# koide3/hdl_graph_slam

Hardware: AMD Instinct MI355X
Metric: registrations/sec (64-beam ~120k-pt pair), loop-closure batch (higher is better)
Workload: dtype f64; 1 GPU; loop-closure batch: 64 candidate keyframes/GPU x HDL-64E (~118848 pts) vs 1 query keyframe, FAST_GICP + getFitnessScore, cold (index + covariances rebuilt every step); candidate set: SURVEY 8d (distinct ray-casts at poses within 20 m of the query, guess = ground truth + 0.5 m / 2 deg noise, z forced to 0); candidates_per_gpu=64, points_per_cloud=118848, method=FAST_GICP, distinct_scans=16, parallelism=single GPU

## Files before the change

### hdl_graph_slam_amd/_lib.py

```python
from __future__ import annotations

import ctypes as C
import os

import numpy as np

_HERE = os.path.dirname(os.path.abspath(__file__))
LIB_PATH = os.path.join(_HERE, "lib", "libhgs_hip.so")

HGS_OK = 0
HGS_ERR_INVALID_ARGUMENT, HGS_ERR_NO_TARGET, HGS_ERR_NO_SOURCE, HGS_ERR_HIP, HGS_ERR_NO_DEVICE, HGS_ERR_UNSUPPORTED, HGS_ERR_OUT_OF_MEMORY, HGS_ERR_INTERNAL, HGS_ERR_COMM = range(1, 10)
HGS_FAST_GICP, HGS_FAST_VGICP, HGS_NDT_OMP, HGS_ICP = 0, 1, 2, 3
HGS_KDTREE, HGS_DIRECT1, HGS_DIRECT7, HGS_DIRECT27 = 0, 1, 2, 3
HGS_REG_FROBENIUS, HGS_REG_PLANE, HGS_REG_MIN_EIG, HGS_REG_NORMALIZED_MIN_EIG, HGS_REG_NONE = 0, 1, 2, 3, 4
STAGES = ["upload", "index", "covariance", "voxelize", "linearize", "error", "solve", "fitness", "prefilter"]
DBL_MAX = float(np.finfo(np.float64).max)

STATUS = {1: "invalid argument", 2: "no target set", 3: "no source set", 4: "HIP runtime error", 5: "no usable HIP device", 6: "unsupported",
          7: "out of host memory inside the backend", 8: "internal error (C++ exception caught at the C boundary)", 9: "communicator error (RCCL)"}


class HgsParams(C.Structure):
    _fields_ = [
        ("method", C.c_int32), ("max_iterations", C.c_int32),
        ("transformation_epsilon", C.c_double), ("rotation_epsilon", C.c_double),
        ("max_correspondence_distance", C.c_double),
        ("correspondence_randomness", C.c_int32), ("neighbor_search", C.c_int32),
        ("resolution", C.c_double), ("ndt_step_size", C.c_double), ("ndt_outlier_ratio", C.c_double),
        ("ndt_min_points_per_voxel", C.c_int32), ("ndt_upstream_hd1_sign", C.c_int32),
        ("lm_max_iterations", C.c_int32), ("lm_init_lambda_factor", C.c_double),
        ("device_id", C.c_int32), ("regularization_method", C.c_int32),
        ("ndt_line_search", C.c_int32), ("reserved", C.c_int32),
    ]

    @property
    def use_reciprocal_correspondences(self) -> bool:
        return bool(self.reserved)

    @use_reciprocal_correspondences.setter
    def use_reciprocal_correspondences(self, on: bool) -> None:
        self.reserved = 1 if on else 0


class HgsPrefilterParams(C.Structure):
    _fields_ = [
        ("use_distance_filter", C.c_int32), ("downsample_method", C.c_int32),
        ("distance_near_thresh", C.c_double), ("distance_far_thresh", C.c_double), ("downsample_resolution", C.c_double),
        ("outlier_removal_method", C.c_int32), ("statistical_mean_k", C.c_int32),
        ("statistical_stddev", C.c_double), ("radius_radius", C.c_double),
        ("radius_min_neighbors", C.c_int32), ("reserved", C.c_int32),
    ]


class HgsPrefilterSweep(C.Structure):
    _fields_ = [
        ("pts", C.c_void_p), ("n", C.c_size_t), ("stride_bytes", C.c_size_t),
        ("imu_angular_velocity", C.c_void_p), ("scan_period", C.c_double), ("sensor_to_base", C.c_void_p),
    ]


class HgsFloorParams(C.Structure):
    _fields_ = [
        ("tilt_deg", C.c_double), ("sensor_height", C.c_double), ("height_clip_range", C.c_double),
        ("floor_pts_thresh", C.c_int32), ("use_normal_filtering", C.c_int32),
        ("floor_normal_thresh", C.c_double), ("normal_filter_thresh", C.c_double),
        ("normal_k", C.c_int32), ("ransac_max_iterations", C.c_int32),
        ("ransac_distance_threshold", C.c_double), ("ransac_probability", C.c_double),
        ("seed", C.c_uint32), ("reserved", C.c_int32),
    ]


class HgsFloorResult(C.Structure):
    _fields_ = [
        ("coeffs", C.c_float * 4), ("detected", C.c_int32), ("reason", C.c_int32),
        ("n_clipped", C.c_uint32), ("n_filtered", C.c_uint32), ("n_inliers", C.c_uint32), ("ransac_iterations", C.c_int32),
    ]


HGS_FLOOR_DETECTED, HGS_FLOOR_TOO_FEW_POINTS, HGS_FLOOR_TOO_FEW_INLIERS, HGS_FLOOR_NOT_VERTICAL = 0, 1, 2, 3
HGS_DOWNSAMPLE_NONE, HGS_DOWNSAMPLE_VOXELGRID, HGS_DOWNSAMPLE_APPROX_VOXELGRID = 0, 1, 2
HGS_OUTLIER_NONE, HGS_OUTLIER_STATISTICAL, HGS_OUTLIER_RADIUS = 0, 1, 2


class HgsResult(C.Structure):
    _fields_ = [
        ("final_transformation", C.c_float * 16), ("converged", C.c_int32), ("iterations", C.c_int32),
        ("error", C.c_double), ("fitness_score", C.c_double), ("num_inliers", C.c_uint32),
        ("candidate_id", C.c_int32), ("lm_tries", C.c_int32), ("reserved", C.c_int32),
    ]

    def matrix(self) -> np.ndarray:
        return np.array(self.final_transformation, dtype=np.float32).reshape(4, 4).T.copy()


RESULT_DTYPE = np.dtype([("final_transformation", "<f4", (16,)), ("converged", "<i4"), ("iterations", "<i4"), ("error", "<f8"),
                         ("fitness_score", "<f8"), ("num_inliers", "<u4"), ("candidate_id", "<i4"), ("lm_tries", "<i4"), ("reserved", "<i4")])
assert RESULT_DTYPE.itemsize == C.sizeof(HgsResult)

EXPORTS = [
    "hgs_params_default", "hgs_create", "hgs_destroy", "hgs_last_error", "hgs_abi_version",
    "hgs_cloud_create", "hgs_cloud_destroy", "hgs_cloud_size", "hgs_cloud_device_bytes", "hgs_cloud_invalidate",
    "hgs_set_target", "hgs_set_target_cloud", "hgs_set_source", "hgs_set_source_cloud",
    "hgs_align", "hgs_transform_source", "hgs_fitness", "hgs_nn_target",
    "hgs_loop_match_batch", "hgs_loop_match_groups", "hgs_align_pairs", "hgs_select_best", "hgs_calc_fitness_score", "hgs_calc_fitness_score_batch",
    "hgs_comm_get_unique_id", "hgs_comm_init", "hgs_comm_finalize", "hgs_loop_match_batch_sharded",
    "hgs_prefilter_params_default", "hgs_prefilter", "hgs_prefilter_deskewed", "hgs_prefilter_framed", "hgs_prefilter_batch", "hgs_cloud_download", "hgs_map_cloud_generate",
    "hgs_floor_params_default", "hgs_detect_floor", "hgs_debug_floor_filter", "hgs_debug_floor_ransac_counts",
    "hgs_profile_enable", "hgs_profile_read", "hgs_synchronize",
    "hgs_debug_target_covariances", "hgs_debug_gicp_linearize", "hgs_debug_icp_correspond", "hgs_debug_icp_step", "hgs_debug_ndt_cells", "hgs_debug_vgicp_voxels", "hgs_debug_cloud_seed_grid", "hgs_debug_ndt_derivatives", "hgs_debug_merge_shard_records", "hgs_debug_set_option",
]

_lib = None


def lib():
    global _lib
    if _lib is not None:
        return _lib
    if not os.path.exists(LIB_PATH):
        raise RuntimeError(f"{LIB_PATH} is missing: build the MI355X backend first (python -c 'import __graft_entry__ as g; g.build()'). "
                           "hdl_graph_slam_amd has no CPU fallback.")
    L = C.CDLL(LIB_PATH)
    vp, sz, fp = C.c_void_p, C.c_size_t, C.POINTER(C.c_float)
    L.hgs_params_default.argtypes = [C.c_int32, C.POINTER(HgsParams)]
    L.hgs_create.argtypes = [C.POINTER(HgsParams), C.POINTER(vp)]
    L.hgs_destroy.argtypes = [vp]
    L.hgs_last_error.argtypes = [vp]
    L.hgs_last_error.restype = C.c_char_p
    L.hgs_cloud_create.argtypes = [vp, vp, sz, sz, C.POINTER(vp)]
    L.hgs_cloud_destroy.argtypes = [vp]
    L.hgs_cloud_size.argtypes = [vp]
    L.hgs_cloud_size.restype = sz
    L.hgs_cloud_device_bytes.argtypes = [vp]
    L.hgs_cloud_device_bytes.restype = sz
    L.hgs_cloud_invalidate.argtypes = [vp]
    L.hgs_set_target.argtypes = [vp, vp, sz, sz]
    L.hgs_set_source.argtypes = [vp, vp, sz, sz]
    L.hgs_set_target_cloud.argtypes = [vp, vp]
    L.hgs_set_source_cloud.argtypes = [vp, vp]
    L.hgs_align.argtypes = [vp, fp, C.POINTER(HgsResult)]
    L.hgs_transform_source.argtypes = [vp, fp, vp, sz]
    L.hgs_fitness.argtypes = [vp, fp, C.c_double, C.POINTER(C.c_double), C.POINTER(C.c_uint32)]
    L.hgs_nn_target.argtypes = [vp, vp, sz, sz, vp, vp]
    L.hgs_loop_match_batch.argtypes = [vp, C.POINTER(vp), sz, vp, C.c_double, vp, C.POINTER(C.c_int32)]
    L.hgs_loop_match_groups.argtypes = [vp, C.POINTER(vp), sz, vp, C.POINTER(vp), vp, C.c_double, vp, vp]
    L.hgs_align_pairs.argtypes = [vp, C.POINTER(vp), C.POINTER(vp), vp, C.POINTER(C.c_double), sz, vp]
    L.hgs_select_best.argtypes = [vp, sz, C.POINTER(C.c_int32)]
    L.hgs_comm_get_unique_id.argtypes = [vp]
    L.hgs_comm_init.argtypes = [vp, C.c_int32, C.c_int32, vp]
    L.hgs_comm_finalize.argtypes = [vp]
    L.hgs_loop_match_batch_sharded.argtypes = [vp, C.POINTER(vp), sz, vp, vp, sz, C.c_double, vp, C.POINTER(C.c_int32)]
    L.hgs_calc_fitness_score.argtypes = [vp, vp, vp, fp, C.c_double, C.POINTER(C.c_double)]
    L.hgs_calc_fitness_score_batch.argtypes = [vp, C.POINTER(vp), C.POINTER(vp), vp, sz, C.c_double, vp, vp]
    L.hgs_prefilter_params_default.argtypes = [C.POINTER(HgsPrefilterParams)]
    L.hgs_prefilter.argtypes = [vp, vp, sz, sz, C.POINTER(HgsPrefilterParams), C.POINTER(vp)]
    L.hgs_prefilter_deskewed.argtypes = [vp, vp, sz, sz, C.POINTER(HgsPrefilterParams), vp, C.c_double, C.POINTER(vp)]
    L.hgs_prefilter_framed.argtypes = [vp, vp, sz, sz, C.POINTER(HgsPrefilterParams), vp, C.c_double, fp, C.POINTER(vp)]
    L.hgs_prefilter_batch.argtypes = [vp, C.POINTER(HgsPrefilterSweep), sz, C.POINTER(HgsPrefilterParams), C.POINTER(vp)]
    L.hgs_cloud_download.argtypes = [vp, vp, sz]
    L.hgs_map_cloud_generate.argtypes = [vp, C.POINTER(vp), vp, sz, C.c_double, C.POINTER(vp)]
    L.hgs_floor_params_default.argtypes = [C.POINTER(HgsFloorParams)]
    L.hgs_detect_floor.argtypes = [vp, vp, C.POINTER(HgsFloorParams), C.POINTER(HgsFloorResult), C.POINTER(vp), C.POINTER(vp)]
    L.hgs_debug_floor_filter.argtypes = [vp, vp, C.POINTER(HgsFloorParams), vp, vp, vp]
    L.hgs_debug_floor_ransac_counts.argtypes = [vp, vp, C.POINTER(HgsFloorParams), C.c_uint32, C.c_uint32, vp, vp]
    L.hgs_profile_enable.argtypes = [vp, C.c_int]
    L.hgs_profile_read.argtypes = [vp, vp, vp, C.c_int]
    L.hgs_synchronize.argtypes = [vp]
    L.hgs_debug_target_covariances.argtypes = [vp, vp]
    L.hgs_debug_set_option.argtypes = [vp, C.c_char_p, C.c_int32]
    L.hgs_debug_gicp_linearize.argtypes = [vp, vp, vp, vp, vp, vp]
    L.hgs_debug_icp_correspond.argtypes = [vp, vp, vp, vp]
    L.hgs_debug_icp_step.argtypes = [vp, vp, vp, C.c_double, C.c_int32, vp, vp, vp]
    L.hgs_debug_ndt_cells.argtypes = [vp, C.c_int32, vp, vp, vp, vp, C.POINTER(C.c_int32)]
    L.hgs_debug_vgicp_voxels.argtypes = [vp, C.c_int32, vp, vp, vp, vp, C.POINTER(C.c_int32)]
    L.hgs_debug_cloud_seed_grid.argtypes = [vp, vp, vp, sz, C.POINTER(C.c_int32), C.POINTER(sz)]
    L.hgs_debug_ndt_derivatives.argtypes = [vp, vp, vp, vp, vp]
    L.hgs_debug_merge_shard_records.argtypes = [vp, vp, C.c_int32, C.c_size_t, C.c_size_t, vp, vp]
    _lib = L
    return L


def default_params(method: int) -> HgsParams:
    p = HgsParams()
    rc = lib().hgs_params_default(method, C.byref(p))
    if rc != HGS_OK:
        raise ValueError(f"hgs_params_default({method}) -> {STATUS.get(rc, rc)}")
    return p


def cloud_args(cloud: np.ndarray):
    cloud = np.ascontiguousarray(cloud)
    if cloud.dtype.fields is not None:
        return cloud, len(cloud), cloud.dtype.itemsize
    cloud = np.ascontiguousarray(cloud, dtype=np.float32)
    if cloud.ndim != 2 or cloud.shape[1] < 3:
        raise ValueError("expected [n, >=3] float32 or PointXYZI records")
    return cloud, cloud.shape[0], cloud.shape[1] * 4


def colmajor16(T) -> np.ndarray:
    return np.ascontiguousarray(np.asarray(T, dtype=np.float32).reshape(4, 4).T.reshape(16))


def fptr(a: np.ndarray):
    return a.ctypes.data_as(C.POINTER(C.c_float))
```

### hdl_graph_slam_amd/csrc/hgs_device.h

```cpp
#pragma once
#include <hip/hip_runtime.h>
#include "hgs_gicp.h"
#include "hgs_floor.h"
#include "hgs_icp.h"
#include "hgs_ndt.h"
#include "hgs_vgicp.h"

namespace hgs {

struct CloudMeta {
  int nvalid;
  int ndt_ncells;
  unsigned bbmin[3];
  unsigned bbmax[3];
  int ndt_min_b[3], ndt_max_b[3], ndt_div_mul[3];
  int ndt_error;
  int vg_ncells;
  int vg_min_b[3], vg_max_b[3], vg_div_mul[3];
  int vg_error;
  int pad[1];
};

struct CloudDesc {
  const float4* raw;
  float4* pts;
  float4* lpts;
  float4* nodes;
  float4* cov;
  int* corr;
  CloudMeta* meta;
  int n_input;
  int P;
  int sort_off;
  int pad;
};

struct TargetView {
  const float4* nodes;
  const float4* pts;
  const float4* lpts;
  const float4* cov;
  const CloudMeta* meta;
  int P;
  int seed_bits;
  const unsigned* seed_tab;
};

struct NdtTargetView {
  const int* hash_keys;
  const int* hash_vals;
  const NdtCellRec* cells;
  const CloudMeta* meta;
  const int2* hash_kv;
  int hash_mask;
  float inv_leaf;
};

struct NdtAccum {
  unsigned long long w[kAccNdt * 4];
  unsigned tiles_done;
  unsigned overflow;
  double out[kAccNdt];
};

struct DevResult {
  float T[16];
  int converged, iterations, lm_tries, pad;
  double error;
  double fit_sum;
  unsigned fit_count;
  unsigned pad2;
};

struct Progress {
  int* dev;
  volatile int* host_done;
  volatile int* host_rounds;
  int B;
  int pad;
};

constexpr int kFusedRoundMaxProblems = 4;
constexpr int kBlock = 256;
constexpr int kKnnLaneList = 16;
constexpr int kKnnLeafLog = 128;
constexpr int kNW = 1;
constexpr int kTileNN = kBlock * kNW;

void launch_pack_aos(hipStream_t s, const float4* staged , int n, float4* raw, float* intensity , CloudMeta* meta_to_reset ,
                     const CloudDesc* desc = nullptr , CloudDesc* desc_out = nullptr);
void launch_meta_init(hipStream_t s, const CloudDesc* descs, int ncloud);
void launch_bbox_count(hipStream_t s, const CloudDesc* descs, int ncloud, int max_n);
void launch_hilbert_keys(hipStream_t s, const CloudDesc* descs, int ncloud, int max_n, unsigned long long* keys, unsigned* vals, int drop_bits);
void launch_gather_sorted(hipStream_t s, const CloudDesc* descs, int ncloud, int max_slots, const unsigned* sorted_vals);
void launch_build_tree(hipStream_t s, const CloudDesc* descs, int ncloud, int max_P);
void launch_knn_cov(hipStream_t s, const CloudDesc* descs, int ncloud, int max_n, int k, int qpw, int reg_method, int gather ,
                    double* raw_stage = nullptr );

void launch_gicp_init(hipStream_t s, GicpState* states, const float* guesses, int B, Progress prog);
struct Guess16 {
  float m[16];
};
void launch_gicp_init1(hipStream_t s, GicpState* states, const float* guess_host , Progress prog);
void launch_gicp_linearize(hipStream_t s, const CloudDesc* descs, TargetView tgt, const GicpState* states, GicpConsts c, double* partials, int max_blocks, int B,
                           int qpw);
void launch_gicp_solve(hipStream_t s, const CloudDesc* descs, GicpState* states, GicpConsts c, const double* partials, int max_blocks, int B,
                       int tile_points );
void launch_gicp_error(hipStream_t s, const CloudDesc* descs, TargetView tgt, const GicpState* states, double* partials_err, int max_blocks, int B);
void launch_gicp_linearize_round2(hipStream_t s, const CloudDesc* descs, TargetView tgt, const GicpState* states_in, GicpState* states_out, GicpConsts c, double* partials,
                                  const double* partials_err, int max_blocks , int lin_blocks , int B, int qpw, Progress prog,
                                  DevResult* results, DevResult* early_out );
void launch_gicp_error_round2(hipStream_t s, const CloudDesc* descs, TargetView tgt, const GicpState* states_in, GicpState* states_out, GicpConsts c, const double* partials,
                              double* partials_err, int max_blocks, int err_blocks , int B, int lin_tile_points);
void launch_gicp_decide(hipStream_t s, const CloudDesc* descs, GicpState* states, GicpConsts c, const double* partials_err, int max_blocks, int B, Progress prog);
void launch_gicp_results(hipStream_t s, const GicpState* states, DevResult* out, int B);

void launch_icp_init(hipStream_t s, IcpState* states, const float* guesses, int B, Progress prog);
void launch_icp_correspond(hipStream_t s, const CloudDesc* descs, TargetView tgt, const IcpState* states, IcpConsts c, double* partials, int max_blocks, int B);
void launch_icp_solve(hipStream_t s, const CloudDesc* descs, IcpState* states, IcpConsts c, const double* partials, int max_blocks, int B, Progress prog);
void launch_icp_results(hipStream_t s, const IcpState* states, DevResult* out, int B);

void launch_fitness(hipStream_t s, const CloudDesc* descs, TargetView tgt, const DevResult* poses, double max_range, double* partials, int max_blocks, int B,
                    int use_seed, int qpw);
void launch_fitness_final(hipStream_t s, const CloudDesc* descs, const double* partials, int max_blocks, DevResult* out, int B, int tile_pts);
void launch_gicp_linearize(hipStream_t s, const CloudDesc* descs, const TargetView* tviews, const GicpState* states, GicpConsts c, double* partials, int max_blocks, int B,
                           int qpw);
void launch_gicp_error(hipStream_t s, const CloudDesc* descs, const TargetView* tviews, const GicpState* states, double* partials_err, int max_blocks, int B);
void launch_gicp_linearize_round2(hipStream_t s, const CloudDesc* descs, const TargetView* tviews, const GicpState* states_in, GicpState* states_out, GicpConsts c, double* partials,
                                  const double* partials_err, int max_blocks, int lin_blocks, int B, int qpw, Progress prog, DevResult* results, DevResult* early_out);
void launch_gicp_error_round2(hipStream_t s, const CloudDesc* descs, const TargetView* tviews, const GicpState* states_in, GicpState* states_out, GicpConsts c, const double* partials,
                              double* partials_err, int max_blocks, int err_blocks, int B, int lin_tile_points);
void launch_icp_correspond(hipStream_t s, const CloudDesc* descs, const TargetView* tviews, const IcpState* states, IcpConsts c, double* partials, int max_blocks, int B);
void launch_fitness(hipStream_t s, const CloudDesc* descs, const TargetView* tviews, const DevResult* poses, double max_range, double* partials, int max_blocks, int B,
                    int use_seed, int qpw);
}
struct hgs_result;
namespace hgs {
void launch_results_to_records(hipStream_t s, const DevResult* res, const int* candidate_ids, int n, int n_slots, ::hgs_result* out);
void launch_nn_query(hipStream_t s, TargetView tgt, const float4* q, int nq, int* idx, float* d2);
void launch_seed_grid_build(hipStream_t s, const float4* pts, const CloudMeta* meta, int n_max, unsigned* tab, int bits);
inline size_t seed_grid_entries(int bits) { return ((size_t)1 << bits) + ((size_t)1 << (bits - 2)) + ((size_t)1 << (bits - 4)); }
struct SeedGridJob {
  const float4* pts;
  const CloudMeta* meta;
  unsigned* tab;
  int bits;
  int pad;
};
void launch_seed_grid_build_batch(hipStream_t s, const SeedGridJob* jobs, int njobs, size_t max_entries, int max_n);
void launch_transform(hipStream_t s, const float4* raw, int n, const float* T16_colmajor_dev, float4* out);

void launch_ndt_grid_params(hipStream_t s, CloudDesc desc, float inv_leaf);
void launch_ndt_cell_keys(hipStream_t s, CloudDesc desc, float inv_leaf, unsigned long long* keys, unsigned* vals);
void launch_ndt_build_cells(hipStream_t s, CloudDesc desc, const unsigned long long* sorted_keys, const unsigned* sorted_vals, int min_points,
                            int* hash_keys, int* hash_vals, int hash_mask, NdtCellRec* cells);
void launch_ndt_init(hipStream_t s, NdtState* states, NdtAngles* angles, const float* guesses, NdtConsts c, int B, Progress prog, NdtAccum* accum_to_zero );
void launch_ndt_pack_hash(hipStream_t s, const int* keys, const int* vals, int2* kv, int cap);
void launch_ndt_pass(hipStream_t s, const CloudDesc* descs, NdtTargetView tgt, NdtState* states, NdtAngles* angles, NdtConsts c, NdtAccum* accum, const int* tile_base,
                     unsigned long long* queues, int B, int parity, int blocks, int chunk, int sorted, int debug, Progress prog);
void launch_ndt_pass(hipStream_t s, const CloudDesc* descs, const NdtTargetView* tviews, NdtState* states, NdtAngles* angles, NdtConsts c, NdtAccum* accum, const int* tile_base,
                     unsigned long long* queues, int B, int parity, int blocks, int chunk, int sorted, int debug, Progress prog);
void launch_ndt_results(hipStream_t s, const CloudDesc* descs, const NdtState* states, DevResult* out, int B);

void launch_vgicp_grid_params(hipStream_t s, CloudDesc desc, double resolution);
void launch_vgicp_cell_keys(hipStream_t s, CloudDesc desc, double resolution, unsigned long long* keys, unsigned* vals);
void launch_vgicp_build_cells(hipStream_t s, CloudDesc desc, const unsigned long long* sorted_keys, const unsigned* sorted_vals, int* hash_keys,
                              int* hash_vals, int hash_mask, NdtCellRec* cells);
void launch_vgicp_linearize(hipStream_t s, const CloudDesc* descs, NdtTargetView tgt, const GicpState* states, VgicpConsts c, double* partials,
                            int max_blocks, int B);
void launch_vgicp_error(hipStream_t s, const CloudDesc* descs, NdtTargetView tgt, const GicpState* states, VgicpConsts c, double* partials_err,
                        int max_blocks, int B);
void launch_vgicp_linearize(hipStream_t s, const CloudDesc* descs, const NdtTargetView* tviews, const GicpState* states, VgicpConsts c, double* partials,
                            int max_blocks, int B);
void launch_vgicp_error(hipStream_t s, const CloudDesc* descs, const NdtTargetView* tviews, const GicpState* states, VgicpConsts c, double* partials_err,
                        int max_blocks, int B);

struct MapSource {
  const float4* raw;
  const float* intensity;
  int n, offset;
  float T[16];
};
void launch_map_transform(hipStream_t s, const MapSource* srcs, int nsrc, int max_n, float4* out);
constexpr int kMapMaxDepth = 21;
constexpr int kMapMaxEvents = kMapMaxDepth + 3;
struct MapOctreeEvent {
  int index, depth;
  double mn[3];
  unsigned long long gained[3];
};
struct MapOctree {
  int first;
  int next_viol;
  int n_events, overflow, done, pad;
  double mx[3];
  MapOctreeEvent events[kMapMaxEvents];
};
void launch_map_first_finite(hipStream_t s, const float4* pts, int n, MapOctree* oct);
void launch_map_octree_init(hipStream_t s, const float4* pts, int n, double res, MapOctree* oct);
void launch_map_octree_step(hipStream_t s, const float4* pts, int n, double res, MapOctree* oct);
void launch_map_keys(hipStream_t s, const float4* pts, int n, double res, const MapOctree* oct, unsigned long long* keys, unsigned* vals);
void launch_map_centers(hipStream_t s, const unsigned long long* keys, const unsigned* head, const unsigned* slot, int n, double res, const MapOctree* oct, float4* out,
                        int* count_out);

struct PfFrame {
  float rows[12];
};
void launch_pf_load(hipStream_t s, const float4* staged, int n, float4* out, const float* deskew_w , double scan_period,
                    const PfFrame* frame , int* count_out, unsigned* meta_out );
void launch_pf_distance_flags(hipStream_t s, const float4* pts, int n, int use_filter, double near_thresh, double far_thresh, unsigned* keep);
void launch_pf_compact(hipStream_t s, const float4* in, int n, const unsigned* keep, const unsigned* slot, float4* out, int* count);
void launch_pf_bbox(hipStream_t s, const float4* pts, const int* count, int cap, unsigned* meta, int dist_filter = 0, double near_thresh = 0, double far_thresh = 0);
void launch_pf_grid(hipStream_t s, unsigned* meta, float inv_leaf);
void launch_pf_voxel_keys(hipStream_t s, const float4* pts, const int* count, const unsigned* meta, float inv_leaf, int cap, unsigned long long* keys, unsigned* vals,
                          int dist_filter = 0, double near_thresh = 0, double far_thresh = 0);
void launch_pf_voxel_heads(hipStream_t s, const unsigned long long* keys, int cap, unsigned* head, unsigned long long invalid_key);
constexpr unsigned long long kVoxelInvalidKey = 0xffffffffull;
constexpr unsigned long long kMapInvalidKey = ~0ull;
void launch_pf_voxel_centroids(hipStream_t s, const float4* pts, const unsigned long long* keys, const unsigned* vals, const unsigned* head, const unsigned* slot, int cap,
                               float4* out, int* count_out, unsigned* ukeys = nullptr );
void launch_pf_grid_radius_flags(hipStream_t s, const float4* cen, const int* count, const unsigned* ukeys, const unsigned* meta, float inv_leaf, float radius, float r2,
                                 int min_neighbors, int cap, unsigned* keep);
void launch_pf_approx_keys(hipStream_t s, const float4* pts, const int* count, float inv_leaf, int cap, unsigned long long* keys, unsigned* vals);
void launch_pf_approx_heads(hipStream_t s, const float4* pts, const unsigned long long* keys, const unsigned* vals, float inv_leaf, int cap, unsigned* head, unsigned* evict,
                            unsigned* bucket_used , unsigned* bucket_rank );
void launch_pf_approx_centroids(hipStream_t s, const float4* pts, const unsigned long long* keys, const unsigned* vals, const unsigned* head, const unsigned* evict,
                                const unsigned* evict_rank, const unsigned* bucket_rank, int cap, float4* out, int* count_out);
void launch_pf_radius_flags(hipStream_t s, CloudDesc d, float r2, int min_neighbors, unsigned* keep);
void launch_pf_mean_knn_dist(hipStream_t s, CloudDesc d, int mean_k, double* dist);
void launch_pf_statistical(hipStream_t s, CloudDesc d, const double* dist, double* stats, double stddev_mul, unsigned* keep);
void launch_pf_to_cloud(hipStream_t s, const float4* in, int n, float4* raw, float* intensity, CloudMeta* meta_to_reset, const CloudDesc* desc = nullptr, CloudDesc* desc_out = nullptr);

struct PfSweep {
  int off, n;
  int count;
  int deskew, frame;
  float w[3];
  double scan_period;
  float rows[12];
  unsigned meta[16];
};
constexpr int kPfBatchOrdinalBits = 12;
void launch_pfb_load(hipStream_t s, const float4* staged, PfSweep* sweeps, int nsweeps, int max_n, float4* out);
void launch_pfb_distance_flags(hipStream_t s, const float4* pts, const PfSweep* sweeps, int nsweeps, int max_n, double near_thresh, double far_thresh, unsigned* keep);
void launch_pfb_compact(hipStream_t s, const float4* in, PfSweep* sweeps, int nsweeps, int max_n, const unsigned* keep, const unsigned* slot, float4* out);
void launch_pfb_bbox(hipStream_t s, const float4* pts, PfSweep* sweeps, int nsweeps, int max_n, int dist_filter, double near_thresh, double far_thresh);
void launch_pfb_grid(hipStream_t s, PfSweep* sweeps, int nsweeps, float inv_leaf);
void launch_pfb_voxel_keys(hipStream_t s, const float4* pts, const PfSweep* sweeps, int nsweeps, int max_n, float inv_leaf, unsigned long long* keys, unsigned* vals,
                           int dist_filter, double near_thresh, double far_thresh);
void launch_pfb_voxel_heads(hipStream_t s, const unsigned long long* keys, const PfSweep* sweeps, int nsweeps, int max_n, unsigned* head);
void launch_pfb_voxel_centroids(hipStream_t s, const float4* pts, const unsigned long long* keys, const unsigned* vals, const unsigned* head, const unsigned* slot,
                                PfSweep* sweeps, int nsweeps, int max_n, float4* out, unsigned* ukeys );
void launch_pfb_grid_radius_flags(hipStream_t s, const float4* cen, const unsigned* ukeys, const PfSweep* sweeps, int nsweeps, int max_n, float inv_leaf, float radius,
                                  float r2, int min_neighbors, unsigned* keep);
void launch_pfb_to_cloud(hipStream_t s, const float4* in, const PfSweep* sweeps, const CloudDesc* descs, CloudDesc* const* desc_outs, float* const* intensities, int nsweeps,
                         int max_m);

void launch_floor_clip_flags(hipStream_t s, const float4* raw, const float* intensity, int n, FloorConsts c, float4* out , unsigned* keep);
void launch_knn_cov_raw(hipStream_t s, const CloudDesc* descs , int max_n, int k, int qpw, int gather, double* raw_stage );
void launch_floor_normal_flags(hipStream_t s, CloudDesc d, const double* raw_cov, FloorConsts c, unsigned* keep , double* normals );
void launch_floor_ransac_init(hipStream_t s, FloorRansacState* st, int max_iterations, Progress prog);
void launch_floor_ransac_planes(hipStream_t s, const float4* pts, int n, unsigned seed, int i0, int nh, const FloorRansacState* st , double* planes ,
                                int* counts );
void launch_floor_ransac_count(hipStream_t s, const float4* pts, int n, double thresh, const double* planes, int nh, const FloorRansacState* st , int* counts);
void launch_floor_ransac_decide(hipStream_t s, const int* counts, const double* planes, int i0, int nh, int n, int max_iterations, double log_prob, FloorRansacState* st,
                                Progress prog);
void launch_floor_inlier_flags(hipStream_t s, const float4* pts, int n, const FloorRansacState* st, double thresh, unsigned* keep);

void launch_gicp_debug_state(hipStream_t s, GicpState* st, const double* T12_dev);
void launch_ndt_debug_state(hipStream_t s, NdtState* st, NdtAngles* ang, const double* p6_dev, NdtConsts c);
void launch_reduce_partials(hipStream_t s, const double* partials, int ntiles, int width , double* out);

}
```

### hdl_graph_slam_amd/csrc/hgs_engine.hip

```cpp
#include <hip/hip_runtime.h>
#include <algorithm>
#include <atomic>
#include <chrono>
#include <climits>
#include <condition_variable>
#include <cmath>
#include <cstdio>
#include <cstdlib>
#include <cstring>
#include <exception>
#include <limits>
#include <mutex>
#include <new>
#include <stdexcept>
#include <string>
#include <thread>
#include <vector>

#include "../../include/hgs_registration.h"
#include "hgs_comm.h"
#include "hgs_consts.h"
#include "hgs_device.h"
#include "hgs_resources.h"
#include "hgs_sort.h"

using namespace hgs;

namespace {

thread_local std::string g_create_error;


int next_pow2(int v) {
  int p = 1;
  while (p < v) p <<= 1;
  return p;
}
size_t align_up(size_t v, size_t a) { return (v + a - 1) / a * a; }

}

struct VoxelTable {
  DeviceBuffer block;
  int* hash_keys = nullptr;
  int* hash_vals = nullptr;
  int2* hash_kv = nullptr;
  NdtCellRec* cells = nullptr;
  int hash_cap = 0;
};

struct hgs_cloud {
  hgs_handle* owner = nullptr;
  size_t n_input = 0;
  int P = 1;
  DeviceBuffer block;
  CloudDesc desc{};
  CloudDesc* dev_desc = nullptr;
  float* intensity = nullptr;
  bool has_index = false;
  bool corr_stale = false;
  bool has_cov = false;
  int cov_k = 0;
  bool has_ndt = false;
  double ndt_resolution = 0;
  int ndt_min_points = 0;
  VoxelTable ndt;
  bool has_vg = false;
  double vg_resolution = 0;
  int vg_cov_k = 0;
  long long vg_span[3] = {0, 0, 0};
  bool vg_too_large = false;
  VoxelTable vg;
  bool has_seed = false;
  DeviceBuffer seed_block;
  int seed_bits = 0;
};

struct ProfEvent {
  int stage;
  hipEvent_t a, b;
};

struct hgs_handle {
  hgs_params prm{};
  int device = 0;
  hipStream_t stream = nullptr;
  hipStream_t lane_stream[7] = {};
  hipEvent_t lane_event[8] = {};
  int lane_start = 1;
  int nn_qpw = 0;
  int nn_qpw16_below = 96, nn_qpw32_below = 0;
  int hilbert_levels = 13;
  hipEvent_t comm_event = nullptr;
  int prefilter_fast = 1;
  int upload_trace = 0;
  int floor_chunk = 64;
  int early_run_ahead = 2;
  int early_result = 1;
  PinnedBuffer h_early;
  hipEvent_t early_event = nullptr;
  bool early_pending = false, early_valid = false;
  int fused_rounds = 1;
  int fused_rounds_below = 262144;
  int fused_rounds_max_problems = kFusedRoundMaxProblems, fused_rounds_max_blocks = 640;
  int cov_split = 1;
  int resident_descs = 1;
  int knn_qpw_tiny = -1;
  int knn_tiny_below = 32768;
  int seed_grid = 1;
  int knn_replay = -1;
  int batch_lanes = 0;
  std::string err;
  hgs_cloud* target = nullptr;
  hgs_cloud* source = nullptr;
  bool own_target = false, own_source = false;
  float final_T[16];

  DeviceBuffer staging, sort_keys[2], sort_vals[2], sort_tmp, descs, states, angles, partials, partials_err, results, guesses, done, misc;
  DeviceBuffer lane_partials[7], lane_partials_err[7];
  DeviceBuffer ndt_accum;
  DeviceBuffer group_tviews, group_corr;
  DeviceBuffer group_vviews;
  DeviceBuffer seed_jobs;
  int pair_chunk = 0;
  hgs::Comm* comm = nullptr;
  DeviceBuffer comm_send, comm_recv, comm_ids;
  DeviceBuffer pf_ukeys;
  DeviceBuffer cov_raw;
  DeviceBuffer ndt_plan;
  int ndt_resident_blocks = 0;
  int ndt_chunk = 0;
  int ndt_sort = -1;
  DeviceBuffer pf_a, pf_b, pf_keep, pf_slot, pf_small, pf_dist;
  DeviceBuffer pf_table;
  PinnedBuffer h_pf_table;
  PinnedBuffer h_results, h_small, h_flags, h_comm;
  PinnedRing up;
  PinnedRing up_points;
  PinnedBuffer up_big;
  hipEvent_t up_big_event = nullptr;
  bool up_big_pending = false;
  PackPool pack_pool;
  PinnedBuffer h_xform;

  std::vector<DeviceBuffer> block_pool;
  std::vector<hgs_cloud*> live_clouds;
  std::recursive_mutex api_mutex;

  bool profiling = false;
  std::vector<ProfEvent> prof_events;
  std::vector<ProfEvent> prof_free;
  double prof_ms[HGS_STAGE_COUNT];
  uint64_t prof_launches[HGS_STAGE_COUNT];

  hgs_handle() = default;
  hgs_handle(const hgs_handle&) = delete;
  hgs_handle& operator=(const hgs_handle&) = delete;
  void synchronize_streams() {
    if (stream) (void)hipStreamSynchronize(stream);
    for (hipStream_t ls : lane_stream)
      if (ls) (void)hipStreamSynchronize(ls);
  }
  ~hgs_handle();
};

namespace {

#define HGS_HIP(h, call)                                                                                           \
  do {                                                                                                             \
    hipError_t e__ = (call);                                                                                       \
    if (e__ != hipSuccess) {                                                                                       \
      char buf__[512];                                                                                             \
      snprintf(buf__, sizeof(buf__), "%s failed: %s (%s:%d)", #call, hipGetErrorString(e__), __FILE__, __LINE__);  \
      (h)->err = buf__;                                                                                            \
      return HGS_ERR_HIP;                                                                                          \
    }                                                                                                              \
  } while (0)

#define HGS_TRY(expr)             \
  do {                            \
    int rc__ = (expr);            \
    if (rc__ != HGS_OK) return rc__; \
  } while (0)

struct StageTimer {
  hgs_handle* h;
  ProfEvent ev{};
  bool active = false;
  StageTimer(hgs_handle* h_, int stage) : h(h_) {
    if (!h->profiling) return;
    if (!h->prof_free.empty()) {
      ev = h->prof_free.back();
      h->prof_free.pop_back();
    } else {
      if (hipEventCreate(&ev.a) != hipSuccess || hipEventCreate(&ev.b) != hipSuccess) return;
    }
    ev.stage = stage;
    active = hipEventRecord(ev.a, h->stream) == hipSuccess;
  }
  ~StageTimer() {
    if (!active) return;
    (void)hipEventRecord(ev.b, h->stream);
    h->prof_events.push_back(ev);
  }
};

struct ApiLock {
  std::unique_lock<std::recursive_mutex> lk;
  explicit ApiLock(hgs_handle* h) {
    if (h) lk = std::unique_lock<std::recursive_mutex>(h->api_mutex);
  }
  explicit ApiLock(hgs_cloud* c) : ApiLock(c ? c->owner : nullptr) {}
};

int set_device(hgs_handle* h) {
  HGS_HIP(h, hipSetDevice(h->device));
  return HGS_OK;
}

constexpr size_t kUploadChunkPoints = 16384;
#ifndef HGS_UPLOAD_PARALLEL_POINTS
#define HGS_UPLOAD_PARALLEL_POINTS 49152
#endif
constexpr size_t kUploadParallelPoints = HGS_UPLOAD_PARALLEL_POINTS;
int upload_image_open(hgs_handle* h, size_t records) {
  if (h->up_big_pending) {
    HGS_HIP(h, hipEventSynchronize(h->up_big_event));
    h->up_big_pending = false;
  }
  HGS_HIP(h, h->up_big.reserve(records * sizeof(float4)));
  return HGS_OK;
}
int upload_image_close(hgs_handle* h) {
  if (!h->up_big_event) HGS_HIP(h, hipEventCreateWithFlags(&h->up_big_event, hipEventDisableTiming));
  HGS_HIP(h, hipEventRecord(h->up_big_event, h->stream));
  h->up_big_pending = true;
  return HGS_OK;
}
int upload_points_at(hgs_handle* h, const void* pts, size_t n, size_t stride_bytes, size_t off, bool in_image) {
  const bool has_intensity = stride_bytes >= 20;
  const char* src = static_cast<const char*>(pts);
  float4* const dev = h->staging.as<float4>() + off;
  if (n >= kUploadParallelPoints) {
    if (!in_image) HGS_TRY(upload_image_open(h, n));
    float4* const image = h->up_big.as<float4>() + (in_image ? off : 0);
    const size_t nchunks = (n + kUploadChunkPoints - 1) / kUploadChunkPoints;
    std::vector<std::atomic<unsigned char>> ready(nchunks);
    for (auto& r : ready) r.store(0, std::memory_order_relaxed);
    PackPool::Job job;
    job.src = src, job.dst = reinterpret_cast<float*>(image), job.n = n, job.stride = stride_bytes, job.chunk = kUploadChunkPoints, job.nchunks = nchunks;
    job.has_intensity = has_intensity, job.ready = ready.data();
    h->pack_pool.post(&job);
    hipError_t err = hipSuccess;
    for (size_t c = 0; c < nchunks; c++) {
      while (!ready[c].load(std::memory_order_acquire))
        if (!PackPool::help(job)) std::this_thread::yield();
      const size_t i0 = c * kUploadChunkPoints, m = std::min(kUploadChunkPoints, n - i0);
      if (err == hipSuccess) err = hipMemcpyAsync(dev + i0, image + i0, m * sizeof(float4), hipMemcpyHostToDevice, h->stream);
    }
    h->pack_pool.retire();
    HGS_HIP(h, err);
    if (!in_image) HGS_TRY(upload_image_close(h));
    return HGS_OK;
  }
  for (size_t i0 = 0; i0 < n; i0 += kUploadChunkPoints) {
    const size_t m = std::min(kUploadChunkPoints, n - i0);
    void* staged = nullptr;
    int slot = 0;
    HGS_HIP(h, h->up_points.stage(kUploadChunkPoints * sizeof(float4), &staged, &slot));
    float* dst = static_cast<float*>(staged);
    const char* s0 = src + i0 * stride_bytes;
    if (has_intensity) {
      for (size_t i = 0; i < m; i++) {
        const float* f = reinterpret_cast<const float*>(s0 + i * stride_bytes);
        dst[4 * i] = f[0], dst[4 * i + 1] = f[1], dst[4 * i + 2] = f[2], dst[4 * i + 3] = f[4];
      }
    } else {
      for (size_t i = 0; i < m; i++) {
        const float* f = reinterpret_cast<const float*>(s0 + i * stride_bytes);
        dst[4 * i] = f[0], dst[4 * i + 1] = f[1], dst[4 * i + 2] = f[2], dst[4 * i + 3] = 0.f;
      }
    }
    HGS_HIP(h, hipMemcpyAsync(dev + i0, staged, m * sizeof(float4), hipMemcpyHostToDevice, h->stream));
    HGS_HIP(h, h->up_points.commit(slot, h->stream));
  }
  return HGS_OK;
}
int upload_points_packed(hgs_handle* h, const void* pts, size_t n, size_t stride_bytes, const float4** dev) {
  HGS_HIP(h, h->staging.reserve(std::max<size_t>(n, 1) * sizeof(float4)));
  *dev = h->staging.as<float4>();
  return upload_points_at(h, pts, n, stride_bytes, 0, false);
}

int cloud_alloc(hgs_handle* h, size_t n, hgs_cloud** out) {
  hgs_cloud* c = new hgs_cloud();
  c->owner = h;
  c->n_input = n;
  c->P = next_pow2((int)((n + kLeaf - 1) / kLeaf));
  if (c->P < 1) c->P = 1;
  const size_t slots = (size_t)c->P * kLeaf;
  const size_t n_cap = align_up(std::max<size_t>(n, 1), 8192);
  size_t off = 0;
  const size_t o_meta = off;
  off = align_up(off + sizeof(CloudMeta), 256);
  const size_t o_desc = off;
  off = align_up(off + sizeof(CloudDesc), 256);
  const size_t o_raw = off;
  off = align_up(off + n_cap * sizeof(float4), 256);
  const size_t o_pts = off;
  off = align_up(off + slots * sizeof(float4), 256);
  const size_t o_lpts = off;
  off = align_up(off + slots * sizeof(float4), 256);
  const size_t o_nodes = off;
// ... 239 lines not shown
      [&](unsigned long long* keys, unsigned* vals) { launch_ndt_build_cells(h->stream, c->desc, keys, vals, min_pts, t.hash_keys, t.hash_vals, cap - 1, t.cells); }));
  launch_ndt_pack_hash(h->stream, t.hash_keys, t.hash_vals, t.hash_kv, cap);
  HGS_HIP(h, hipGetLastError());
  c->has_ndt = true;
  c->ndt_resolution = res;
  c->ndt_min_points = min_pts;
  return HGS_OK;
}

int vgicp_grid_too_large(hgs_handle* h, const hgs_cloud* c) {
  char msg[256];
  snprintf(msg, sizeof(msg),
           "FAST_VGICP: the target's voxel grid spans %lld x %lld x %lld cells at resolution %g, more than the 2147483647 a linear voxel key addresses "
           "(a far stray point in the target?)",
           c->vg_span[0], c->vg_span[1], c->vg_span[2], c->vg_resolution);
  h->err = msg;
  return HGS_ERR_UNSUPPORTED;
}

int ensure_vgicp_target(hgs_handle* h, hgs_cloud* c) {
  const double res = h->prm.resolution;
  const int k = h->prm.correspondence_randomness;
  if (c->has_vg && c->vg_resolution == res && c->vg_cov_k == cov_cache_key(h, k)) return c->vg_too_large ? vgicp_grid_too_large(h, c) : HGS_OK;
  StageTimer tm(h, HGS_STAGE_VOXELIZE);
  const int max_cells = (int)c->n_input + 1;
  const int cap = next_pow2(std::max<int>(64, 2 * max_cells));
  VoxelTable& t = c->vg;
  HGS_TRY(build_voxel_table(
      h, c, t, cap, max_cells, false, [&] { launch_vgicp_grid_params(h->stream, c->desc, res); },
      [&](unsigned long long* keys, unsigned* vals) { launch_vgicp_cell_keys(h->stream, c->desc, res, keys, vals); },
      [&](unsigned long long* keys, unsigned* vals) { launch_vgicp_build_cells(h->stream, c->desc, keys, vals, t.hash_keys, t.hash_vals, cap - 1, t.cells); }));
  HGS_HIP(h, hipGetLastError());
  HGS_HIP(h, h->h_small.reserve(sizeof(CloudMeta)));
  const CloudMeta* hm = h->h_small.as<CloudMeta>();
  HGS_HIP(h, hipMemcpyAsync(h->h_small.p, c->desc.meta, sizeof(CloudMeta), hipMemcpyDeviceToHost, h->stream));
  HGS_HIP(h, hipStreamSynchronize(h->stream));
  for (int d = 0; d < 3; d++) c->vg_span[d] = (long long)hm->vg_max_b[d] - hm->vg_min_b[d] + 1;
  c->vg_too_large = hm->vg_error != 0;
  c->has_vg = true;
  c->vg_resolution = res;
  c->vg_cov_k = cov_cache_key(h, k);
  return c->vg_too_large ? vgicp_grid_too_large(h, c) : HGS_OK;
}

NdtTargetView voxel_target_view(const hgs_cloud* c, const VoxelTable& t, float inv_leaf) {
  NdtTargetView tv;
  tv.hash_keys = t.hash_keys, tv.hash_vals = t.hash_vals, tv.cells = t.cells, tv.meta = c->desc.meta, tv.hash_kv = t.hash_kv;
  tv.hash_mask = t.hash_cap - 1, tv.inv_leaf = inv_leaf;
  return tv;
}
NdtTargetView ndt_target_view(const hgs_handle* h, const hgs_cloud* t) { return voxel_target_view(t, t->ndt, 1.0f / (float)h->prm.resolution); }
NdtTargetView vgicp_target_view(const hgs_cloud* t) { return voxel_target_view(t, t->vg, 0.f); }

TargetView target_view(const hgs_cloud* c) {
  TargetView t;
  t.nodes = c->desc.nodes, t.pts = c->desc.pts, t.lpts = c->desc.lpts, t.cov = c->desc.cov, t.meta = c->desc.meta, t.P = c->P;
  t.seed_bits = c->has_seed ? c->seed_bits : 0, t.seed_tab = c->has_seed ? c->seed_block.as<const unsigned>() : nullptr;
  return t;
}

int ensure_seed_grid(hgs_handle* h, hgs_cloud* c) {
  if (!h->seed_grid || c->has_seed || !c->has_index || c->n_input == 0) return HGS_OK;
  int bits = 12;
  while (bits < 24 && ((size_t)1 << bits) < 4 * c->n_input) bits++;
  const size_t bytes = seed_grid_entries(bits) * sizeof(unsigned);
  if (!c->seed_block.p || c->seed_bits != bits) {
    HGS_HIP(h, c->seed_block.alloc(bytes));
    c->seed_bits = bits;
  }
  HGS_HIP(h, hipMemsetAsync(c->seed_block.p, 0xff, bytes, h->stream));
  launch_seed_grid_build(h->stream, c->desc.pts, c->desc.meta, (int)c->n_input, c->seed_block.as<unsigned>(), bits);
  HGS_HIP(h, hipGetLastError());
  c->has_seed = true;
  return HGS_OK;
}

int ensure_seed_grids(hgs_handle* h, const std::vector<hgs_cloud*>& all) {
  if (!h->seed_grid) return HGS_OK;
  std::vector<hgs_cloud*> todo;
  for (hgs_cloud* c : all)
    if (!c->has_seed && c->has_index && c->n_input > 0 && std::find(todo.begin(), todo.end(), c) == todo.end()) todo.push_back(c);
  constexpr size_t kMaxJobs = 65535;
  for (size_t start = 0; start < todo.size(); start += kMaxJobs) {
    const size_t nj = std::min(kMaxJobs, todo.size() - start);
    std::vector<SeedGridJob> jobs(nj);
    size_t max_entries = 0;
    int max_n = 0;
    for (size_t j = 0; j < nj; j++) {
      hgs_cloud* c = todo[start + j];
      int bits = 12;
      while (bits < 24 && ((size_t)1 << bits) < 4 * c->n_input) bits++;
      const size_t entries = seed_grid_entries(bits);
      if (!c->seed_block.p || c->seed_bits != bits) {
        HGS_HIP(h, c->seed_block.alloc(entries * sizeof(unsigned)));
        c->seed_bits = bits;
      }
      jobs[j] = SeedGridJob{c->desc.pts, c->desc.meta, c->seed_block.as<unsigned>(), bits, 0};
      max_entries = std::max(max_entries, entries), max_n = std::max(max_n, (int)c->n_input);
    }
    HGS_HIP(h, h->seed_jobs.reserve(nj * sizeof(SeedGridJob)));
    HGS_HIP(h, h->up.upload(h->seed_jobs.p, jobs.data(), nj * sizeof(SeedGridJob), h->stream));
    launch_seed_grid_build_batch(h->stream, h->seed_jobs.as<SeedGridJob>(), (int)nj, max_entries, max_n);
    HGS_HIP(h, hipGetLastError());
    for (size_t j = 0; j < nj; j++) todo[start + j]->has_seed = true;
  }
  return HGS_OK;
}

NdtConsts engine_ndt_consts(const hgs_params& p) {
  NdtConsts c = ndt_consts(p);
  c.pad = std::getenv("HGS_TRACE") ? 1 : 0;
  return c;
}

constexpr int kMaxCountedDevices = 64;
std::atomic<int> g_streams_in_use[kMaxCountedDevices] = {};
std::atomic<int>& streams_in_use(int device) { return g_streams_in_use[(unsigned)device % kMaxCountedDevices]; }
int hw_queue_budget() {
  static const int budget = [] {
    const char* e = std::getenv("GPU_MAX_HW_QUEUES");
    const int v = e ? std::atoi(e) : 0;
    return v > 0 ? v : 4;
  }();
  return budget;
}
constexpr int kFloorMaxChunk = 4096;
constexpr int kMaxLanes = 8;

int make_progress(hgs_handle* h, int lane, int B, Progress* out) {
  if (h->early_pending) {
    HGS_HIP(h, hipEventSynchronize(h->early_event));
    h->early_pending = false;
  }
  HGS_HIP(h, h->done.reserve(64));
  HGS_HIP(h, h->h_flags.reserve(64));
  volatile int* hf = h->h_flags.as<volatile int>() + 2 * lane;
  hf[0] = 0, hf[1] = 0;
  out->dev = h->done.as<int>() + 2 * lane;
  out->host_done = hf, out->host_rounds = hf + 1;
  out->B = B, out->pad = 0;
  return HGS_OK;
}

struct BatchLane {
  hipStream_t stream = nullptr;
  int b0 = 0, B = 0;
  Progress prog{};
  double* partials = nullptr;
  double* partials_err = nullptr;
  long round = 0;
  bool finished = false;
};

int open_lanes(hgs_handle* h, int B, size_t partial_bytes_per_problem, size_t partial_err_bytes_per_problem, std::vector<BatchLane>& lanes, int tiles_per_problem) {
  const bool small_problems = tiles_per_problem > 0 && tiles_per_problem <= 96;
  const int by_size = h->prm.method == HGS_NDT_OMP ? (B > 32 && !small_problems ? 3 : 4) : (small_problems && (long)B * tiles_per_problem <= 3072 ? 1 : 4);
  const int wanted = h->batch_lanes > 0 ? h->batch_lanes : by_size;
  int n = h->profiling ? 1 : std::max(1, std::min(std::min(wanted, kMaxLanes), B));
  if (h->batch_lanes <= 0) {
    int owned = 0;
    while (owned < kMaxLanes - 1 && h->lane_stream[owned]) owned++;
    const int room = std::max(0, hw_queue_budget() - streams_in_use(h->device).load(std::memory_order_relaxed));
    n = std::min(n, 1 + owned + room);
  }
  lanes.assign(n, BatchLane{});
  for (int i = 0, b0 = 0; i < n; i++) {
    BatchLane& L = lanes[i];
    L.b0 = b0, L.B = (B - b0) / (n - i);
    b0 += L.B;
    HGS_TRY(make_progress(h, i, L.B, &L.prog));
    if (i == 0) {
      L.stream = h->stream;
      L.partials = h->partials.as<double>(), L.partials_err = h->partials_err.as<double>();
      continue;
    }
    if (!h->lane_stream[i - 1]) {
      HGS_HIP(h, hipStreamCreateWithFlags(&h->lane_stream[i - 1], hipStreamNonBlocking));
      streams_in_use(h->device).fetch_add(1, std::memory_order_relaxed);
    }
    L.stream = h->lane_stream[i - 1];
    HGS_HIP(h, h->lane_partials[i - 1].reserve((size_t)L.B * partial_bytes_per_problem));
    HGS_HIP(h, h->lane_partials_err[i - 1].reserve((size_t)L.B * partial_err_bytes_per_problem));
    L.partials = h->lane_partials[i - 1].as<double>(), L.partials_err = h->lane_partials_err[i - 1].as<double>();
  }
  if (n > 1) {
    if (h->lane_start != 0) HGS_HIP(h, hipStreamSynchronize(h->stream));
    if (!h->lane_event[0]) HGS_HIP(h, hipEventCreateWithFlags(&h->lane_event[0], hipEventDisableTiming));
    HGS_HIP(h, hipEventRecord(h->lane_event[0], h->stream));
    for (int i = 1; i < n; i++) HGS_HIP(h, hipStreamWaitEvent(lanes[i].stream, h->lane_event[0], 0));
  }
  return HGS_OK;
}

int close_lanes(hgs_handle* h, std::vector<BatchLane>& lanes) {
  for (size_t i = 1; i < lanes.size(); i++) {
    if (!h->lane_event[i]) HGS_HIP(h, hipEventCreateWithFlags(&h->lane_event[i], hipEventDisableTiming));
    HGS_HIP(h, hipEventRecord(h->lane_event[i], lanes[i].stream));
    HGS_HIP(h, hipStreamWaitEvent(h->stream, h->lane_event[i], 0));
  }
  return HGS_OK;
}

constexpr long kRunAhead = 2;
template <typename F, typename G>
void drive_lanes(std::vector<BatchLane>& lanes, long max_rounds, F&& enqueue_round, G&& on_finished, long run_ahead = kRunAhead) {
  long spins = 0;
  for (;;) {
    bool all_finished = true, enqueued = false;
    for (BatchLane& L : lanes) {
      if (L.finished) continue;
      if (*L.prog.host_done || L.round >= max_rounds) {
        L.finished = true;
        on_finished(L);
        continue;
      }
      all_finished = false;
      if (L.round - (long)*L.prog.host_rounds < run_ahead) {
        enqueue_round(L);
        L.round++;
        enqueued = true;
      }
    }
    if (all_finished) return;
    if (enqueued) {
      spins = 0;
      continue;
    }
    if ((++spins & 0x3ff) == 0) {
      for (BatchLane& L : lanes)
        if (!L.finished && !*L.prog.host_done && hipStreamQuery(L.stream) == hipSuccess && !*L.prog.host_done &&
            L.round - (long)*L.prog.host_rounds >= run_ahead) {
          enqueue_round(L);
          L.round++;
        }
    }
#if defined(__x86_64__)
    __builtin_ia32_pause();
#endif
  }
}

struct BatchShape {
  int B, max_n;
  int qpw, nn_tile;
  bool gicp_round2;
  int lin_qpw, lin_tile, lin_blocks;
  int max_blocks, err_blocks;
  const CloudDesc* d_descs;
  const TargetView* d_tviews;
  const NdtTargetView* d_vviews;
};

template <typename F>
void with_lane_target(const BatchShape& s, const BatchLane& L, const TargetView& tv, F&& launch) {
  if (s.d_tviews) launch(s.d_tviews + L.b0);
  else launch(tv);
}

int batch_shape(hgs_handle* h, const std::vector<hgs_cloud*>& sources, bool lm_rounds, BatchShape* out, int* const* corr_of = nullptr) {
  BatchShape& s = *out;
  s.d_tviews = nullptr, s.d_vviews = nullptr;
  s.B = (int)sources.size();
  s.max_n = 0;
  for (hgs_cloud* c : sources) s.max_n = std::max(s.max_n, (int)c->n_input);
  const int B = s.B, max_n = s.max_n;
  s.qpw = 64;
  s.nn_tile = (kBlock / 64) * s.qpw * kNW;
  s.gicp_round2 = lm_rounds && h->prm.method == HGS_FAST_GICP && h->fused_rounds && max_n <= h->fused_rounds_below &&
                  (B <= h->fused_rounds_max_problems || (long)B * ((max_n + kBlock - 1) / kBlock) <= (long)h->fused_rounds_max_blocks);
  const long tiles64 = (long)B * ((max_n + s.nn_tile - 1) / s.nn_tile);
  s.lin_qpw = !s.gicp_round2 ? 64 : h->nn_qpw > 0 ? h->nn_qpw : tiles64 <= (long)h->nn_qpw16_below ? 16 : tiles64 <= (long)h->nn_qpw32_below ? 32 : 64;
  s.lin_tile = (kBlock / 64) * s.lin_qpw * kNW;
  s.lin_blocks = std::max(1, (max_n + s.lin_tile - 1) / s.lin_tile);
  s.max_blocks = std::max(1, s.lin_qpw < 64 ? (max_n + 63) / 64 : (max_n + s.nn_tile - 1) / s.nn_tile);
  s.err_blocks = std::max(1, (max_n + kBlock - 1) / kBlock);
  return upload_descs(h, sources, false, &s.d_descs, nullptr, corr_of);
}

bool corr_seeds_fitness(int method) { return method == HGS_FAST_GICP || method == HGS_ICP; }
void lane_fitness(hgs_handle* h, BatchLane& L, const BatchShape& s, double max_range, bool corr_seeds) {
  StageTimer tm(h, HGS_STAGE_FITNESS);
  DevResult* res = h->results.as<DevResult>() + L.b0;
  with_lane_target(s, L, s.d_tviews ? TargetView{} : target_view(h->target),
                   [&](auto tgt) { launch_fitness(L.stream, s.d_descs + L.b0, tgt, res, max_range, L.partials_err, s.max_blocks, L.B, corr_seeds ? 1 : 0, s.qpw); });
  launch_fitness_final(L.stream, s.d_descs + L.b0, L.partials_err, s.max_blocks, res, L.B, s.nn_tile);
}
void lane_fitness_tail(hgs_handle* h, BatchLane& L, const BatchShape& s, const double* fit_max_range) {
  if (fit_max_range) lane_fitness(h, L, s, *fit_max_range, corr_seeds_fitness(h->prm.method));
}

int run_gicp_rounds(hgs_handle* h, const BatchShape& s, const float* guesses_host, bool guess_in_args, const double* fit_max_range) {
  const int B = s.B, max_blocks = s.max_blocks;
  hgs_cloud* tgt = h->target;
  const bool voxel = h->prm.method == HGS_FAST_VGICP;
  const GicpConsts c = gicp_consts(h->prm);
  const VgicpConsts vc = vgicp_consts(h->prm);
  const bool round2 = s.gicp_round2;
  const bool early = round2 && B == 1 && !fit_max_range && h->early_result && !h->profiling;
  DevResult* early_out = nullptr;
  if (early) {
    HGS_HIP(h, h->h_early.reserve(sizeof(DevResult)));
    early_out = h->h_early.as<DevResult>();
  }
  HGS_HIP(h, h->states.reserve((size_t)B * sizeof(GicpState) * (round2 ? 2 : 1)));
  GicpState* st = h->states.as<GicpState>();
  GicpState* st_other = st + B;
  const TargetView tv = s.d_tviews || s.d_vviews ? TargetView{} : target_view(tgt);
  const NdtTargetView vtv = voxel && !s.d_vviews ? vgicp_target_view(tgt) : NdtTargetView{};
  const long max_rounds = (long)std::max(1, c.max_iterations) * std::max(1, c.lm_max_iterations) + 2 + (round2 ? 1 : 0);
  std::vector<BatchLane> lanes;
  HGS_TRY(open_lanes(h, B, (size_t)max_blocks * kAccNdt * sizeof(double), (size_t)max_blocks * 2 * sizeof(double), lanes, s.err_blocks));
  auto finish_lane = [&](BatchLane& L) {
    if (early && *L.prog.host_done) {
      h->early_valid = true;
      return;
    }
    launch_gicp_results(L.stream, st + L.b0, h->results.as<DevResult>() + L.b0, L.B);
    lane_fitness_tail(h, L, s, fit_max_range);
  };
  if (guess_in_args) launch_gicp_init1(lanes[0].stream, st, guesses_host, lanes[0].prog);
  else
    for (BatchLane& L : lanes) launch_gicp_init(L.stream, st + L.b0, h->guesses.as<float>() + (size_t)L.b0 * 16, L.B, L.prog);
  drive_lanes(lanes, max_rounds, [&](BatchLane& L) {
    const CloudDesc* dd = s.d_descs + L.b0;
    GicpState* ls = st + L.b0;
    if (round2) {
      {
        StageTimer tm(h, HGS_STAGE_LINEARIZE);
        with_lane_target(s, L, tv, [&](auto t) {
          launch_gicp_linearize_round2(L.stream, dd, t, ls, st_other + L.b0, c, L.partials, L.partials_err, max_blocks, s.lin_blocks, L.B, s.lin_qpw, L.prog,
                                       h->results.as<DevResult>() + L.b0, early_out);
        });
      }
      StageTimer tm(h, HGS_STAGE_ERROR);
      with_lane_target(s, L, tv, [&](auto t) {
        launch_gicp_error_round2(L.stream, dd, t, st_other + L.b0, ls, c, L.partials, L.partials_err, max_blocks, s.err_blocks, L.B, s.lin_tile);
      });
      return;
    }
    {
      StageTimer tm(h, HGS_STAGE_LINEARIZE);
      if (voxel && s.d_vviews) launch_vgicp_linearize(L.stream, dd, s.d_vviews + L.b0, ls, vc, L.partials, max_blocks, L.B);
      else if (voxel) launch_vgicp_linearize(L.stream, dd, vtv, ls, vc, L.partials, max_blocks, L.B);
      else with_lane_target(s, L, tv, [&](auto t) { launch_gicp_linearize(L.stream, dd, t, ls, c, L.partials, max_blocks, L.B, s.qpw); });
    }
    {
      StageTimer tm(h, HGS_STAGE_SOLVE);
      launch_gicp_solve(L.stream, dd, ls, c, L.partials, max_blocks, L.B, voxel ? kBlock : s.nn_tile);
    }
    {
      StageTimer tm(h, HGS_STAGE_ERROR);
      if (voxel && s.d_vviews) launch_vgicp_error(L.stream, dd, s.d_vviews + L.b0, ls, vc, L.partials_err, max_blocks, L.B);
      else if (voxel) launch_vgicp_error(L.stream, dd, vtv, ls, vc, L.partials_err, max_blocks, L.B);
      else with_lane_target(s, L, tv, [&](auto t) { launch_gicp_error(L.stream, dd, t, ls, L.partials_err, max_blocks, L.B); });
    }
    {
      StageTimer tm(h, HGS_STAGE_SOLVE);
      launch_gicp_decide(L.stream, dd, ls, c, L.partials_err, max_blocks, L.B, L.prog);
    }
  }, finish_lane, early ? (long)h->early_run_ahead : kRunAhead);
  HGS_TRY(close_lanes(h, lanes));
  if (h->early_valid) {
    if (!h->early_event) HGS_HIP(h, hipEventCreateWithFlags(&h->early_event, hipEventDisableTiming));
    HGS_HIP(h, hipEventRecord(h->early_event, h->stream));
    h->early_pending = true;
  }
  return HGS_OK;
}

int run_icp_rounds(hgs_handle* h, const BatchShape& s, const double* fit_max_range) {
  const int B = s.B, max_blocks = s.max_blocks;
  const IcpConsts c = icp_consts(h->prm);
  HGS_HIP(h, h->states.reserve((size_t)B * sizeof(IcpState)));
  IcpState* st = h->states.as<IcpState>();
  const TargetView tv = s.d_tviews ? TargetView{} : target_view(h->target);
  const long max_rounds = (long)std::max(0, c.max_iterations) + 2;
  std::vector<BatchLane> lanes;
  HGS_TRY(open_lanes(h, B, (size_t)max_blocks * kAccIcp * sizeof(double), (size_t)max_blocks * 2 * sizeof(double), lanes, s.err_blocks));
  auto finish_lane = [&](BatchLane& L) {
    launch_icp_results(L.stream, st + L.b0, h->results.as<DevResult>() + L.b0, L.B);
    lane_fitness_tail(h, L, s, fit_max_range);
  };
  for (BatchLane& L : lanes) launch_icp_init(L.stream, st + L.b0, h->guesses.as<float>() + (size_t)L.b0 * 16, L.B, L.prog);
  drive_lanes(lanes, max_rounds, [&](BatchLane& L) {
    {
      StageTimer tm(h, HGS_STAGE_LINEARIZE);
      with_lane_target(s, L, tv, [&](auto t) { launch_icp_correspond(L.stream, s.d_descs + L.b0, t, st + L.b0, c, L.partials, max_blocks, L.B); });
    }
    StageTimer tm(h, HGS_STAGE_SOLVE);
    launch_icp_solve(L.stream, s.d_descs + L.b0, st + L.b0, c, L.partials, max_blocks, L.B, L.prog);
  }, finish_lane);
  return close_lanes(h, lanes);
}

struct NdtLanePlan {
  int* tile_base;
  unsigned long long* queues;
  int blocks, chunk;
};
int ndt_lane_plans(hgs_handle* h, const std::vector<hgs_cloud*>& sources, const std::vector<BatchLane>& lanes, std::vector<NdtLanePlan>& plans) {
  plans.assign(lanes.size(), NdtLanePlan{});
  const size_t per_lane = align_up(16 + (sources.size() + 1) * sizeof(int), 256);
  bool tile_overflow = false;
  constexpr long long kMaxNdtBlocks = 1 << 16, kMaxNdtChunk = 1 << 10;
  HGS_HIP(h, h->ndt_plan.reserve(per_lane * lanes.size()));
  void* staged = nullptr;
  int plan_slot = 0;
  HGS_HIP(h, h->up.stage(per_lane * lanes.size(), &staged, &plan_slot));
  std::memset(staged, 0, per_lane * lanes.size());
  char* const host = static_cast<char*>(staged);
  for (size_t li = 0; li < lanes.size(); li++) {
    const BatchLane& L = lanes[li];
    int* tb = reinterpret_cast<int*>(host + li * per_lane + 16);
    tb[0] = 0;
    long long tiles64 = 0;
    for (int k = 0; k < L.B; k++) {
      tiles64 += std::max<long long>(1, ((long long)sources[L.b0 + k]->n_input + kBlock - 1) / kBlock);
      tile_overflow = tile_overflow || tiles64 > (long long)INT_MAX - (long long)kMaxNdtBlocks * kMaxNdtChunk;
      tb[k + 1] = tile_overflow ? 0 : (int)tiles64;
    }
    NdtLanePlan& P = plans[li];
    const int total = tb[L.B];
    if (tile_overflow) continue;
    P.blocks = std::max(1, std::min(total, h->ndt_resident_blocks > 0 ? std::min(h->ndt_resident_blocks, (int)kMaxNdtBlocks) : (lanes.size() > 1 ? 512 : 768)));
    P.chunk = h->ndt_chunk > 0 ? std::min(h->ndt_chunk, (int)kMaxNdtChunk) : 8;
    P.queues = reinterpret_cast<unsigned long long*>((char*)h->ndt_plan.p + li * per_lane);
    P.tile_base = reinterpret_cast<int*>((char*)h->ndt_plan.p + li * per_lane + 16);
  }
  if (tile_overflow) {
    h->err = "NDT batch too large: the tiles of one lane do not fit 32-bit item arithmetic (more than ~5e11 source points in one call)";
    return HGS_ERR_INVALID_ARGUMENT;
  }
  HGS_HIP(h, hipMemcpyAsync(h->ndt_plan.p, host, per_lane * lanes.size(), hipMemcpyHostToDevice, h->stream));
  HGS_HIP(h, h->up.commit(plan_slot, h->stream));
  if (lanes.size() > 1) {
    HGS_HIP(h, hipEventRecord(h->lane_event[0], h->stream));
    for (size_t i = 1; i < lanes.size(); i++) HGS_HIP(h, hipStreamWaitEvent(lanes[i].stream, h->lane_event[0], 0));
  }
  return HGS_OK;
}

int run_ndt_rounds(hgs_handle* h, const std::vector<hgs_cloud*>& sources, const BatchShape& s, const double* fit_max_range) {
  const int B = s.B, max_blocks = s.max_blocks;
  const NdtConsts c = engine_ndt_consts(h->prm);
  HGS_HIP(h, h->states.reserve((size_t)B * sizeof(NdtState)));
  HGS_HIP(h, h->angles.reserve((size_t)B * sizeof(NdtAngles)));
  NdtState* st = h->states.as<NdtState>();
  NdtAngles* ang = h->angles.as<NdtAngles>();
  const NdtTargetView tv = s.d_vviews ? NdtTargetView{} : ndt_target_view(h, h->target);
  if (h->ndt_sort == 1) HGS_TRY(ensure_index(h, sources));
  bool sorted = h->ndt_sort != 0;
  for (hgs_cloud* sc : sources) sorted = sorted && sc->has_index;
  HGS_HIP(h, h->ndt_accum.reserve((size_t)B * sizeof(NdtAccum)));
  NdtAccum* accum = h->ndt_accum.as<NdtAccum>();
  const long max_rounds = ((long)c.max_iterations + 4) * (c.line_search ? 11 : 1);
  std::vector<BatchLane> lanes;
  HGS_TRY(open_lanes(h, B, (size_t)max_blocks * 2 * sizeof(double), (size_t)max_blocks * 2 * sizeof(double), lanes, s.err_blocks));
  auto finish_lane = [&](BatchLane& L) {
    launch_ndt_results(L.stream, s.d_descs + L.b0, st + L.b0, h->results.as<DevResult>() + L.b0, L.B);
    lane_fitness_tail(h, L, s, fit_max_range);
  };
  std::vector<NdtLanePlan> plans;
  HGS_TRY(ndt_lane_plans(h, sources, lanes, plans));
  for (BatchLane& L : lanes) launch_ndt_init(L.stream, st + L.b0, ang + L.b0, h->guesses.as<float>() + (size_t)L.b0 * 16, c, L.B, L.prog, accum + L.b0);
  drive_lanes(lanes, max_rounds, [&](BatchLane& L) {
    StageTimer tm(h, HGS_STAGE_LINEARIZE);
    const NdtLanePlan& P = plans[&L - lanes.data()];
    if (s.d_vviews)
      launch_ndt_pass(L.stream, s.d_descs + L.b0, s.d_vviews + L.b0, st + L.b0, ang + L.b0, c, accum + L.b0, P.tile_base, P.queues, L.B, (int)(L.round & 1), P.blocks,
                      P.chunk, sorted ? 1 : 0, 0, L.prog);
    else
      launch_ndt_pass(L.stream, s.d_descs + L.b0, tv, st + L.b0, ang + L.b0, c, accum + L.b0, P.tile_base, P.queues, L.B, (int)(L.round & 1), P.blocks, P.chunk,
                      sorted ? 1 : 0, 0, L.prog);
  }, finish_lane);
  return close_lanes(h, lanes);
}

int run_batch(hgs_handle* h, const std::vector<hgs_cloud*>& sources, const float* guesses_host, const double* fit_max_range = nullptr) {
  const int B = (int)sources.size();
  h->early_valid = false;
  hgs_cloud* tgt = h->target;
  const int method = h->prm.method;
  const bool gicp = method == HGS_FAST_GICP || method == HGS_FAST_VGICP;
  std::vector<hgs_cloud*> all(sources);
  if (fit_max_range) {
    std::vector<hgs_cloud*> searched(sources);
    searched.push_back(tgt);
    HGS_TRY(ensure_index(h, searched));
  }
  if (gicp) {
    all.push_back(tgt);
    HGS_TRY(ensure_cov(h, all, h->prm.correspondence_randomness));
    if (method == HGS_FAST_VGICP) HGS_TRY(ensure_vgicp_target(h, tgt));
  } else if (method == HGS_ICP) {
    all.push_back(tgt);
    HGS_TRY(ensure_index(h, all));
  } else {
    HGS_TRY(ensure_ndt_target(h, tgt));
  }
  if (fit_max_range && method != HGS_FAST_GICP) HGS_TRY(ensure_seed_grid(h, tgt));
  BatchShape s;
  HGS_TRY(batch_shape(h, sources, true, &s));
  const bool guess_in_args = B == 1 && method == HGS_FAST_GICP;
  HGS_HIP(h, h->guesses.reserve((size_t)B * 16 * sizeof(float)));
  if (!guess_in_args) HGS_HIP(h, h->up.upload(h->guesses.p, guesses_host, (size_t)B * 16 * sizeof(float), h->stream));
  HGS_HIP(h, h->results.reserve((size_t)B * sizeof(DevResult)));
  HGS_HIP(h, h->partials.reserve((size_t)B * s.max_blocks * kAccNdt * sizeof(double)));
  HGS_HIP(h, h->partials_err.reserve((size_t)B * s.max_blocks * 2 * sizeof(double)));
  if (gicp) HGS_TRY(run_gicp_rounds(h, s, guesses_host, guess_in_args, fit_max_range));
  else if (method == HGS_ICP) HGS_TRY(run_icp_rounds(h, s, fit_max_range));
  else HGS_TRY(run_ndt_rounds(h, sources, s, fit_max_range));
  HGS_HIP(h, hipGetLastError());
  return HGS_OK;
}

int run_group_batch(hgs_handle* h, const std::vector<hgs_cloud*>& targets, const std::vector<hgs_cloud*>& sources, const float* guesses_host, const double* fit_max_range) {
  const int B = (int)sources.size();
  const int method = h->prm.method;
  h->early_valid = false;
  std::vector<hgs_cloud*> all(sources);
  all.insert(all.end(), targets.begin(), targets.end());
  if (method == HGS_FAST_GICP) HGS_TRY(ensure_cov(h, all, h->prm.correspondence_randomness));
  else HGS_TRY(ensure_index(h, all));
  if (fit_max_range && method != HGS_FAST_GICP)
    for (hgs_cloud* t : targets) HGS_TRY(ensure_seed_grid(h, t));
  std::vector<size_t> corr_off(B + 1, 0);
  for (int b = 0; b < B; b++) corr_off[b + 1] = corr_off[b] + align_up((size_t)sources[b]->P * kLeaf, 64);
  HGS_HIP(h, h->group_corr.reserve(std::max<size_t>(1, corr_off[B]) * sizeof(int)));
  HGS_HIP(h, hipMemsetAsync(h->group_corr.p, 0xff, corr_off[B] * sizeof(int), h->stream));
  std::vector<int*> corr_of(B);
  for (int b = 0; b < B; b++) corr_of[b] = h->group_corr.as<int>() + corr_off[b];
  std::vector<TargetView> views(B);
  for (int b = 0; b < B; b++) views[b] = target_view(targets[b]);
  HGS_HIP(h, h->group_tviews.reserve((size_t)B * sizeof(TargetView)));
  HGS_HIP(h, h->up.upload(h->group_tviews.p, views.data(), (size_t)B * sizeof(TargetView), h->stream));
  BatchShape s;
  HGS_TRY(batch_shape(h, sources, true, &s, corr_of.data()));
  s.d_tviews = h->group_tviews.as<TargetView>();
  HGS_HIP(h, h->guesses.reserve((size_t)B * 16 * sizeof(float)));
  HGS_HIP(h, h->up.upload(h->guesses.p, guesses_host, (size_t)B * 16 * sizeof(float), h->stream));
  HGS_HIP(h, h->results.reserve((size_t)B * sizeof(DevResult)));
  HGS_HIP(h, h->partials.reserve((size_t)B * s.max_blocks * kAccNdt * sizeof(double)));
  HGS_HIP(h, h->partials_err.reserve((size_t)B * s.max_blocks * 2 * sizeof(double)));
  if (method == HGS_FAST_GICP) HGS_TRY(run_gicp_rounds(h, s, guesses_host, false, fit_max_range));
  else HGS_TRY(run_icp_rounds(h, s, fit_max_range));
  HGS_HIP(h, hipGetLastError());
  return HGS_OK;
}

int run_pair_batch(hgs_handle* h, const std::vector<hgs_cloud*>& targets, const std::vector<hgs_cloud*>& sources, const float* guesses_host, const double* fit_max_range) {
  const int method = h->prm.method;
  if (method == HGS_FAST_GICP || method == HGS_ICP) return run_group_batch(h, targets, sources, guesses_host, fit_max_range);
  const int B = (int)sources.size();
  const bool voxel = method == HGS_FAST_VGICP;
  h->early_valid = false;
  std::vector<hgs_cloud*> all(sources);
  all.insert(all.end(), targets.begin(), targets.end());
  std::vector<hgs_cloud*> distinct;
  for (hgs_cloud* t : targets)
    if (std::find(distinct.begin(), distinct.end(), t) == distinct.end()) distinct.push_back(t);
  if (fit_max_range) HGS_TRY(ensure_index(h, all));
  if (voxel) {
    HGS_TRY(ensure_cov(h, all, h->prm.correspondence_randomness));
    for (hgs_cloud* t : distinct) {
      const int rc = ensure_vgicp_target(h, t);
      if (rc == HGS_ERR_UNSUPPORTED) {
        const size_t pair = (size_t)(std::find(targets.begin(), targets.end(), t) - targets.begin());
        h->err = "hgs_align_pairs: pair " + std::to_string(pair) + ": " + h->err;
      }
      HGS_TRY(rc);
    }
  } else {
    for (hgs_cloud* t : distinct) HGS_TRY(ensure_ndt_target(h, t));
  }
  if (fit_max_range) HGS_TRY(ensure_seed_grids(h, distinct));
  std::vector<int*> corr_of;
  if (voxel) {
    std::vector<size_t> corr_off(B + 1, 0);
    for (int b = 0; b < B; b++) corr_off[b + 1] = corr_off[b] + align_up((size_t)sources[b]->P * kLeaf, 64);
    HGS_HIP(h, h->group_corr.reserve(std::max<size_t>(1, corr_off[B]) * sizeof(int)));
    HGS_HIP(h, hipMemsetAsync(h->group_corr.p, 0xff, corr_off[B] * sizeof(int), h->stream));
    corr_of.resize(B);
    for (int b = 0; b < B; b++) corr_of[b] = h->group_corr.as<int>() + corr_off[b];
  }
  std::vector<NdtTargetView> vviews(B);
  for (int b = 0; b < B; b++) vviews[b] = voxel ? vgicp_target_view(targets[b]) : ndt_target_view(h, targets[b]);
  HGS_HIP(h, h->group_vviews.reserve((size_t)B * sizeof(NdtTargetView)));
  HGS_HIP(h, h->up.upload(h->group_vviews.p, vviews.data(), (size_t)B * sizeof(NdtTargetView), h->stream));
  if (fit_max_range) {
    std::vector<TargetView> views(B);
    for (int b = 0; b < B; b++) views[b] = target_view(targets[b]);
    HGS_HIP(h, h->group_tviews.reserve((size_t)B * sizeof(TargetView)));
    HGS_HIP(h, h->up.upload(h->group_tviews.p, views.data(), (size_t)B * sizeof(TargetView), h->stream));
  }
  BatchShape s;
  HGS_TRY(batch_shape(h, sources, true, &s, voxel ? corr_of.data() : nullptr));
  s.d_vviews = h->group_vviews.as<NdtTargetView>();
  s.d_tviews = fit_max_range ? h->group_tviews.as<TargetView>() : nullptr;
  HGS_HIP(h, h->guesses.reserve((size_t)B * 16 * sizeof(float)));
  HGS_HIP(h, h->up.upload(h->guesses.p, guesses_host, (size_t)B * 16 * sizeof(float), h->stream));
  HGS_HIP(h, h->results.reserve((size_t)B * sizeof(DevResult)));
  HGS_HIP(h, h->partials.reserve((size_t)B * s.max_blocks * kAccNdt * sizeof(double)));
  HGS_HIP(h, h->partials_err.reserve((size_t)B * s.max_blocks * 2 * sizeof(double)));
  if (voxel) HGS_TRY(run_gicp_rounds(h, s, guesses_host, false, fit_max_range));
  else HGS_TRY(run_ndt_rounds(h, sources, s, fit_max_range));
  HGS_HIP(h, hipGetLastError());
  return HGS_OK;
}

int run_fitness(hgs_handle* h, const std::vector<hgs_cloud*>& sources, double max_range, bool use_corr_seeds) {
  std::vector<hgs_cloud*> all(sources);
  all.push_back(h->target);
  HGS_TRY(ensure_index(h, all));
  if (!use_corr_seeds) HGS_TRY(ensure_seed_grid(h, h->target));
  BatchShape s;
  HGS_TRY(batch_shape(h, sources, false, &s));
  HGS_HIP(h, h->partials_err.reserve((size_t)s.B * s.max_blocks * 2 * sizeof(double)));
  BatchLane whole;
  whole.stream = h->stream, whole.B = s.B, whole.partials_err = h->partials_err.as<double>();
  lane_fitness(h, whole, s, max_range, use_corr_seeds);
  HGS_HIP(h, hipGetLastError());
  return HGS_OK;
}

int fetch_results(hgs_handle* h, int B, std::vector<DevResult>& out) {
  HGS_HIP(h, h->h_results.reserve((size_t)B * sizeof(DevResult)));
  HGS_HIP(h, hipMemcpyAsync(h->h_results.p, h->results.p, (size_t)B * sizeof(DevResult), hipMemcpyDeviceToHost, h->stream));
  HGS_HIP(h, hipStreamSynchronize(h->stream));
  out.assign(h->h_results.as<DevResult>(), h->h_results.as<DevResult>() + B);
  return HGS_OK;
}

double fitness_score(const DevResult& d) { return d.fit_count > 0 ? d.fit_sum / (double)d.fit_count : std::numeric_limits<double>::max(); }

int run_pair_fitness(hgs_handle* h, hgs_cloud* const* cloud1, hgs_cloud* const* cloud2, const float* relposes, size_t n_pairs, double max_range,
                     std::vector<DevResult>& out) {
  std::vector<hgs_cloud*> all(cloud2, cloud2 + n_pairs);
  all.insert(all.end(), cloud1, cloud1 + n_pairs);
  HGS_TRY(ensure_index(h, all));
  HGS_TRY(ensure_seed_grids(h, std::vector<hgs_cloud*>(cloud1, cloud1 + n_pairs)));
  const size_t chunk = h->pair_chunk > 0 ? (size_t)h->pair_chunk : 65535;
  out.clear();
  out.reserve(n_pairs);
  for (size_t p0 = 0; p0 < n_pairs; p0 += chunk) {
    const size_t B = std::min(chunk, n_pairs - p0);
    std::vector<TargetView> views(B);
    for (size_t b = 0; b < B; b++) views[b] = target_view(cloud1[p0 + b]);
    HGS_HIP(h, h->group_tviews.reserve(B * sizeof(TargetView)));
    HGS_HIP(h, h->up.upload(h->group_tviews.p, views.data(), B * sizeof(TargetView), h->stream));
    BatchShape s;
    HGS_TRY(batch_shape(h, std::vector<hgs_cloud*>(cloud2 + p0, cloud2 + p0 + B), false, &s));
    s.d_tviews = h->group_tviews.as<TargetView>();
    std::vector<DevResult> poses(B);
    std::memset(poses.data(), 0, B * sizeof(DevResult));
    for (size_t b = 0; b < B; b++) std::memcpy(poses[b].T, relposes + 16 * (p0 + b), sizeof(float) * 16);
    HGS_HIP(h, h->results.reserve(B * sizeof(DevResult)));
    HGS_HIP(h, h->up.upload(h->results.p, poses.data(), B * sizeof(DevResult), h->stream));
    HGS_HIP(h, h->partials_err.reserve(B * s.max_blocks * 2 * sizeof(double)));
    BatchLane whole;
    whole.stream = h->stream, whole.B = (int)B, whole.partials_err = h->partials_err.as<double>();
    lane_fitness(h, whole, s, max_range, false);
    HGS_HIP(h, hipGetLastError());
    std::vector<DevResult> r;
    HGS_TRY(fetch_results(h, (int)B, r));
    out.insert(out.end(), r.begin(), r.end());
  }
  return HGS_OK;
}

void to_public(const DevResult& d, int candidate, bool with_fitness, hgs_result* r) {
  std::memcpy(r->final_transformation, d.T, sizeof(float) * 16);
  r->converged = d.converged;
  r->iterations = d.iterations;
  r->error = d.error;
  r->lm_tries = d.lm_tries;
  r->candidate_id = candidate;
  r->reserved = 0;
  if (with_fitness) {
    r->num_inliers = d.fit_count;
    r->fitness_score = fitness_score(d);
  } else {
    r->num_inliers = 0;
    r->fitness_score = std::numeric_limits<double>::quiet_NaN();
  }
}

int upload_pose_as_result(hgs_handle* h, const float T[16]) {
  HGS_HIP(h, h->results.reserve(sizeof(DevResult)));
  HGS_HIP(h, h->h_results.reserve(sizeof(DevResult)));
  DevResult* r = h->h_results.as<DevResult>();
  std::memset(r, 0, sizeof(DevResult));
  std::memcpy(r->T, T, sizeof(float) * 16);
  HGS_HIP(h, hipMemcpyAsync(h->results.p, r, sizeof(DevResult), hipMemcpyHostToDevice, h->stream));
  return HGS_OK;
}

int status_of_current_exception(hgs_handle* h) noexcept {
  int rc = HGS_ERR_INTERNAL;
  char what[256] = "unknown C++ exception inside the backend";
  try {
    throw;
  } catch (const std::bad_alloc&) {
    rc = HGS_ERR_OUT_OF_MEMORY;
    snprintf(what, sizeof(what), "out of host memory");
  } catch (const std::exception& e) {
    snprintf(what, sizeof(what), "C++ exception inside the backend: %s", e.what());
  } catch (...) {
  }
  try {
    if (h) h->err = what;
    else g_create_error = what;
  } catch (...) {
  }
  return rc;
}

int set_role_cloud(hgs_handle* h, hgs_cloud* c, hgs_cloud* hgs_handle::*role, bool hgs_handle::*own) {
  ApiLock lock(h);
  if (!h || !c || c->owner != h) return HGS_ERR_INVALID_ARGUMENT;
  if (h->*own && h->*role != c) cloud_free(h->*role);
  h->*role = c;
  h->*own = false;
  return HGS_OK;
}
int set_role_points(hgs_handle* h, const void* pts, size_t n, size_t stride_bytes, hgs_cloud* hgs_handle::*role, bool hgs_handle::*own) {
  ApiLock lock(h);
  if (!h) return HGS_ERR_INVALID_ARGUMENT;
  hgs_cloud* c = nullptr;
  HGS_TRY(hgs_cloud_create(h, pts, n, stride_bytes, &c));
  if (h->*own) cloud_free(h->*role);
  h->*role = c;
  h->*own = true;
  return HGS_OK;
}

}

hgs_handle::~hgs_handle() {
  (void)hipSetDevice(device);
  synchronize_streams();
  pack_pool.shutdown();
  if (comm) hgs::comm_destroy(comm);
  for (hipEvent_t ev : lane_event)
    if (ev) (void)hipEventDestroy(ev);
  for (hipEvent_t ev : {comm_event, early_event, up_big_event})
    if (ev) (void)hipEventDestroy(ev);
  for (const std::vector<ProfEvent>* list : {&prof_events, &prof_free})
    for (const ProfEvent& ev : *list) (void)hipEventDestroy(ev.a), (void)hipEventDestroy(ev.b);
  for (hipStream_t ls : lane_stream)
    if (ls) (void)hipStreamDestroy(ls), streams_in_use(device).fetch_sub(1, std::memory_order_relaxed);
  if (stream) (void)hipStreamDestroy(stream), streams_in_use(device).fetch_sub(1, std::memory_order_relaxed);
}

extern "C" {

int hgs_abi_version(void) { return HGS_ABI_VERSION; }

int hgs_debug_set_option(hgs_handle* h, const char* key, int value) try {
  ApiLock lock(h);
  if (!h || !key) return HGS_ERR_INVALID_ARGUMENT;
  const std::string k(key);
  if (k == "batch_lanes") h->batch_lanes = value <= 0 ? 0 : std::min(kMaxLanes, value);
  else if (k == "lane_start") h->lane_start = value != 0 ? 1 : 0;
  else if (k == "ndt_sort") h->ndt_sort = std::max(-1, std::min(1, value));
  else if (k == "cov_split") h->cov_split = value != 0 ? 1 : 0;
  else if (k == "fused_rounds") h->fused_rounds = value != 0 ? 1 : 0;
  else if (k == "early_result") h->early_result = value != 0 ? 1 : 0;
  else if (k == "early_run_ahead") h->early_run_ahead = std::max(1, std::min(8, value));
  else if (k == "fused_rounds_max_problems") h->fused_rounds_max_problems = std::max(0, value);
  else if (k == "fused_rounds_max_blocks") h->fused_rounds_max_blocks = std::max(0, value);
  else if (k == "fused_rounds_below") h->fused_rounds_below = std::max(0, value);
  else if (k == "resident_descs") h->resident_descs = value != 0 ? 1 : 0;
  else if (k == "knn_qpw_tiny") h->knn_qpw_tiny = value < 0 ? -1 : std::max(0, std::min(32, value & ~7));
  else if (k == "knn_tiny_below") h->knn_tiny_below = std::max(0, value);
  else if (k == "seed_grid") h->seed_grid = value != 0 ? 1 : 0;
  else if (k == "knn_replay") h->knn_replay = std::max(-1, std::min(2, value));
  else if (k == "ndt_resident") h->ndt_resident_blocks = std::max(0, value);
  else if (k == "ndt_chunk") h->ndt_chunk = std::max(0, value);
  else if (k == "hilbert_levels") h->hilbert_levels = std::max(4, std::min(16, value));
  else if (k == "nn_qpw") h->nn_qpw = value == 16 ? 16 : (value == 32 ? 32 : (value == 64 ? 64 : 0));
  else if (k == "nn_qpw16_below") h->nn_qpw16_below = std::max(0, value);
  else if (k == "nn_qpw32_below") h->nn_qpw32_below = std::max(0, value);
  else if (k == "upload_trace") h->upload_trace = value != 0 ? 1 : 0;
  else if (k == "prefilter_fast") h->prefilter_fast = value != 0 ? 1 : 0;
  else if (k == "floor_chunk") h->floor_chunk = std::max(1, std::min(kFloorMaxChunk, value));
  else if (k == "pair_chunk") h->pair_chunk = std::max(0, std::min(65535, value));
  else {
    h->err = "hgs_debug_set_option: unknown option '" + k + "'";
    return HGS_ERR_INVALID_ARGUMENT;
  }
  return HGS_OK;
} catch (...) {
  return status_of_current_exception(h);
}

int hgs_params_default(int32_t method, hgs_params* p) try {
  if (!p || method < HGS_FAST_GICP || method > HGS_ICP) return HGS_ERR_INVALID_ARGUMENT;
  std::memset(p, 0, sizeof(*p));
  p->method = method;
  p->max_iterations = 64;
  p->transformation_epsilon = 0.01;
  p->rotation_epsilon = method == HGS_ICP ? 0.0 : 2e-3;
  p->max_correspondence_distance = method == HGS_FAST_GICP || method == HGS_ICP ? 2.5 : (double)FLT_MAX;
  p->correspondence_randomness = 20;
  p->neighbor_search = method == HGS_NDT_OMP ? HGS_DIRECT7 : HGS_DIRECT1;
  p->resolution = method == HGS_NDT_OMP ? 0.5 : 1.0;
  p->ndt_step_size = 0.1;
  p->ndt_outlier_ratio = 0.55;
  p->ndt_min_points_per_voxel = 6;
  p->ndt_upstream_hd1_sign = 1;
  p->lm_max_iterations = 10;
  p->lm_init_lambda_factor = 1e-9;
  p->device_id = 0;
  p->regularization_method = HGS_REG_FROBENIUS;
  p->ndt_line_search = 0;
  p->icp_reciprocal = 0;
  return HGS_OK;
} catch (...) {
  return status_of_current_exception(nullptr);
}

int hgs_create(const hgs_params* p, hgs_handle** out) try {
  if (!p || !out) return HGS_ERR_INVALID_ARGUMENT;
  *out = nullptr;
  if (p->method < HGS_FAST_GICP || p->method > HGS_ICP || p->max_iterations < 0 || p->correspondence_randomness < 1 || p->correspondence_randomness > 64  || !(p->resolution > 0) ||
      p->regularization_method < HGS_REG_FROBENIUS || p->regularization_method > HGS_REG_NONE) {
    g_create_error = "invalid hgs_params";
    return HGS_ERR_INVALID_ARGUMENT;
  }
  int ndev = 0;
  hipError_t e = hipGetDeviceCount(&ndev);
  if (e != hipSuccess || ndev <= 0 || p->device_id < 0 || p->device_id >= ndev) {
    g_create_error = std::string("no usable HIP device: ") + (e != hipSuccess ? hipGetErrorString(e) : "device ordinal out of range");
    return HGS_ERR_NO_DEVICE;
  }
  hgs_handle* h = new hgs_handle();
  h->prm = *p;
  h->device = p->device_id;
  for (int i = 0; i < 16; i++) h->final_T[i] = (i % 5 == 0) ? 1.f : 0.f;
  for (int i = 0; i < HGS_STAGE_COUNT; i++) h->prof_ms[i] = 0, h->prof_launches[i] = 0;
  if (hipSetDevice(h->device) != hipSuccess || hipStreamCreateWithFlags(&h->stream, hipStreamNonBlocking) != hipSuccess) {
    g_create_error = "hipSetDevice / hipStreamCreate failed";
    delete h;
    return HGS_ERR_HIP;
  }
  streams_in_use(h->device).fetch_add(1, std::memory_order_relaxed);
  *out = h;
  return HGS_OK;
} catch (...) {
  return status_of_current_exception(nullptr);
}

int hgs_destroy(hgs_handle* h) try {
  if (!h) return HGS_OK;
  { std::lock_guard<std::recursive_mutex> wait_for_running_call(h->api_mutex); }
  (void)hipSetDevice(h->device);
  h->synchronize_streams();
  if (h->own_target) cloud_free(h->target);
  if (h->own_source) cloud_free(h->source);
  for (hgs_cloud* c : h->live_clouds) {
    cloud_release_device(c, false);
    c->owner = nullptr;
    c->n_input = 0;
  }
  delete h;
  return HGS_OK;
} catch (...) {
  return status_of_current_exception(nullptr);
}

const char* hgs_last_error(const hgs_handle* h) { return h ? h->err.c_str() : g_create_error.c_str(); }

int hgs_cloud_create(hgs_handle* h, const void* pts, size_t n, size_t stride_bytes, hgs_cloud** out) try {
  ApiLock lock(h);
  if (!h || !out || (n > 0 && !pts) || stride_bytes < 12 || (stride_bytes % 4) != 0 || n > (size_t)1 << 30) return HGS_ERR_INVALID_ARGUMENT;
  HGS_TRY(set_device(h));
  const bool trace = h->upload_trace != 0;
  const auto t0 = std::chrono::steady_clock::now();
  hgs_cloud* c = nullptr;
  HGS_TRY(cloud_alloc(h, n, &c));
  const auto t1 = std::chrono::steady_clock::now();
  auto t2 = t1;
  {
    StageTimer tm(h, HGS_STAGE_UPLOAD);
    const float4* staged = nullptr;
    {
      const int rc = upload_points_packed(h, pts, n, stride_bytes, &staged);
      t2 = std::chrono::steady_clock::now();
      if (rc != HGS_OK) {
        cloud_free(c);
        return rc;
      }
    }
    const CloudDesc resident = resident_desc(c);
    launch_pack_aos(h->stream, staged, (int)n, const_cast<float4*>(c->desc.raw), c->intensity, c->desc.meta, &resident, c->dev_desc);
    launch_bbox_count(h->stream, c->dev_desc, 1, (int)n);
    hipError_t e = hipGetLastError();
    if (e != hipSuccess) {
      h->err = std::string("cloud upload failed: ") + hipGetErrorString(e);
      cloud_free(c);
      return HGS_ERR_HIP;
    }
  }
  if (trace) {
    const auto t3 = std::chrono::steady_clock::now();
    auto us = [](auto a, auto b) { return std::chrono::duration<double, std::micro>(b - a).count(); };
    std::fprintf(stderr, "[hgs upload] n %zu: alloc %.1f us, pack + DMA enqueue %.1f us, launches %.1f us\n", n, us(t0, t1), us(t1, t2), us(t2, t3));
  }
  *out = c;
  return HGS_OK;
} catch (...) {
  return status_of_current_exception(h);
}

int hgs_cloud_destroy(hgs_cloud* c) try {
  ApiLock lock(c);
  if (!c) return HGS_OK;
  hgs_handle* h = c->owner;
  if (h) {
    (void)hipSetDevice(h->device);
    (void)hipStreamSynchronize(h->stream);
    if (h->target == c) h->target = nullptr, h->own_target = false;
    if (h->source == c) h->source = nullptr, h->own_source = false;
  }
  cloud_free(c);
  c = nullptr;
  return HGS_OK;
} catch (...) {
  return status_of_current_exception(nullptr);
}

size_t hgs_cloud_size(const hgs_cloud* c) { return c ? c->n_input : 0; }

size_t hgs_cloud_device_bytes(const hgs_cloud* c) {
  if (!c || !c->owner) return 0;
  return c->block.cap + c->ndt.block.cap + c->vg.block.cap + c->seed_block.cap;
}

int hgs_cloud_invalidate(hgs_cloud* c) try {
  ApiLock lock(c);
  if (!c) return HGS_ERR_INVALID_ARGUMENT;
  c->has_index = false, c->has_cov = false, c->has_ndt = false, c->has_vg = false, c->has_seed = false;
  c->corr_stale = true;
  return HGS_OK;
} catch (...) {
  return status_of_current_exception((c ? c->owner : nullptr));
}

// ... 285 lines not shown
  return status_of_current_exception(nullptr);
}

int hgs_comm_init(hgs_handle* h, int32_t rank, int32_t world, const void* unique_id) try {
  ApiLock lock(h);
  if (!h || !unique_id || world < 1 || rank < 0 || rank >= world) return HGS_ERR_INVALID_ARGUMENT;
  HGS_TRY(set_device(h));
  if (h->comm) hgs::comm_destroy(h->comm), h->comm = nullptr;
  char err[256] = "";
  if (hgs::comm_create(&h->comm, rank, world, unique_id, h->device, err, sizeof(err)) != 0) {
    h->err = err;
    return HGS_ERR_COMM;
  }
  return HGS_OK;
} catch (...) {
  return status_of_current_exception(h);
}

int hgs_comm_finalize(hgs_handle* h) try {
  ApiLock lock(h);
  if (!h) return HGS_ERR_INVALID_ARGUMENT;
  if (h->comm) {
    (void)hipSetDevice(h->device);
    (void)hipStreamSynchronize(h->stream);
    hgs::comm_destroy(h->comm);
    h->comm = nullptr;
  }
  return HGS_OK;
} catch (...) {
  return status_of_current_exception(h);
}

int hgs_debug_merge_shard_records(const hgs_result* gathered, const int32_t* counts, int32_t world, size_t per, size_t n_total, hgs_result* all_out,
                                  int32_t* duplicate_id) try {
  if (!all_out || n_total == 0 || world < 1 || (per > 0 && !gathered) || !counts) return HGS_ERR_INVALID_ARGUMENT;
  for (size_t i = 0; i < n_total; i++) {
    std::memset(&all_out[i], 0, sizeof(hgs_result));
    all_out[i].candidate_id = (int32_t)i;
    all_out[i].fitness_score = std::numeric_limits<double>::max();
  }
  std::vector<char> seen(n_total, 0);
  int32_t dup = -1;
  for (int32_t r = 0; r < world; r++) {
    const size_t n = counts[r] < 0 ? 0 : std::min<size_t>((size_t)counts[r], per);
    for (size_t k = 0; k < n; k++) {
      const hgs_result& rec = gathered[(size_t)r * per + k];
      if (rec.candidate_id < 0 || (size_t)rec.candidate_id >= n_total) continue;
      if (seen[rec.candidate_id]) {
        if (dup < 0) dup = rec.candidate_id;
        continue;
      }
      seen[rec.candidate_id] = 1;
      all_out[rec.candidate_id] = rec;
    }
  }
  if (duplicate_id) *duplicate_id = dup;
  return HGS_OK;
} catch (...) {
  return status_of_current_exception(nullptr);
}

}
namespace {
long comm_timeout_ms() {
  if (const char* e = std::getenv("HGS_COMM_TIMEOUT_MS")) return std::max(0l, std::atol(e));
  return 60000;
}
template <typename Q>
int comm_wait(hgs_handle* h, Q&& query, const char* what) {
  const long limit_ms = comm_timeout_ms();
  const auto t0 = std::chrono::steady_clock::now();
  auto next_check = t0 + std::chrono::milliseconds(1);
  long sleep_us = 0;
  char err[256] = "";
  for (;;) {
    const hipError_t e = query();
    if (e == hipSuccess) return HGS_OK;
    if (e != hipErrorNotReady) {
      h->err = std::string("hgs_loop_match_batch_sharded: HIP error while waiting for ") + what + ": " + hipGetErrorString(e);
      hgs::comm_abort(h->comm);
      return HGS_ERR_HIP;
    }
    const auto now = std::chrono::steady_clock::now();
    if (now >= next_check) {
      next_check = now + std::chrono::milliseconds(1);
      if (hgs::comm_async_error(h->comm, err, sizeof(err)) != 0) {
        h->err = std::string("hgs_loop_match_batch_sharded: the communicator reported an asynchronous error while waiting for ") + what + ": " + err;
        hgs::comm_abort(h->comm);
        return HGS_ERR_COMM;
      }
      const long waited = (long)std::chrono::duration_cast<std::chrono::milliseconds>(now - t0).count();
      if (limit_ms > 0 && waited > limit_ms) {
        h->err = std::string("hgs_loop_match_batch_sharded: gave up after ") + std::to_string(waited) + " ms waiting for " + what +
                 " (a peer has left the collective or never entered it); the communicator has been aborted";
        hgs::comm_abort(h->comm);
        return HGS_ERR_COMM;
      }
    }
    if (now - t0 > std::chrono::microseconds(200)) {
      sleep_us = sleep_us == 0 ? 5 : std::min(50l, sleep_us * 2);
      std::this_thread::sleep_for(std::chrono::microseconds(sleep_us));
    }
  }
}
struct CommAbortGuard {
  hgs::Comm* comm;
  bool armed = true;
  ~CommAbortGuard() {
    if (armed) hgs::comm_abort(comm);
  }
};
#ifdef HGS_TESTING
bool fault_after_header(const char* kind, int rank) {
  const char* e = std::getenv("HGS_FAULT_AFTER_HEADER");
  if (!e) return false;
  const size_t n = std::strlen(kind);
  return std::strncmp(e, kind, n) == 0 && e[n] == ':' && std::atoi(e + n + 1) == rank;
}
#else
constexpr bool fault_after_header(const char*, int) { return false; }
#endif
}
extern "C" {

int hgs_loop_match_batch_sharded(hgs_handle* h, hgs_cloud* const* candidates, size_t n_mine, const int32_t* candidate_ids, const float* guesses,
                                 size_t n_total, double max_range, hgs_result* all_out, int32_t* best) try {
  ApiLock lock(h);
  if (!h || !all_out || n_total == 0 || n_total > (size_t)1 << 24) return HGS_ERR_INVALID_ARGUMENT;
  if (!h->comm) {
    h->err = "hgs_loop_match_batch_sharded: hgs_comm_init has not been called on this engine";
    return HGS_ERR_COMM;
  }
  if (best) *best = -1;
  const int world = hgs::comm_world(h->comm), rank = hgs::comm_rank(h->comm);
  int local = HGS_OK;
  std::string local_err;
  auto fail_local = [&](int rc, const std::string& why) {
    if (local == HGS_OK) local = rc, local_err = why;
  };
  if (n_mine > n_total || (n_mine > 0 && (!candidates || !candidate_ids || !guesses))) fail_local(HGS_ERR_INVALID_ARGUMENT, "hgs_loop_match_batch_sharded: bad candidate arrays");
  if (!h->target) fail_local(HGS_ERR_NO_TARGET, "hgs_loop_match_batch_sharded: no target set on this rank");
  std::vector<hgs_cloud*> src;
  if (local == HGS_OK) {
    src.assign(candidates, candidates + n_mine);
    for (size_t i = 0; i < n_mine; i++)
      if (!src[i] || src[i]->owner != h || candidate_ids[i] < 0 || (size_t)candidate_ids[i] >= n_total)
        fail_local(HGS_ERR_INVALID_ARGUMENT, "hgs_loop_match_batch_sharded: candidate " + std::to_string(i) + " is not a cloud of this engine or its id is out of range");
    std::vector<hgs_cloud*> sorted(src);
    std::sort(sorted.begin(), sorted.end());
    if (std::adjacent_find(sorted.begin(), sorted.end()) != sorted.end()) fail_local(HGS_ERR_INVALID_ARGUMENT, "hgs_loop_match_batch_sharded: candidate clouds must be distinct");
  }
  const size_t n_send = local == HGS_OK ? n_mine : 0;
  const size_t hdr_bytes = 16;
  const size_t ids_off = align_up((size_t)world * hdr_bytes + hdr_bytes, 16), rec_off = align_up(ids_off + n_total * sizeof(int32_t), 16);
  bool mem_ok = set_device(h) == HGS_OK;
  mem_ok = mem_ok && h->results.reserve(std::max<size_t>(n_total, 1) * sizeof(DevResult)) == hipSuccess;
  mem_ok = mem_ok && h->comm_send.reserve(n_total * sizeof(hgs_result) + hdr_bytes) == hipSuccess;
  mem_ok = mem_ok && h->comm_recv.reserve((size_t)world * (n_total * sizeof(hgs_result) + hdr_bytes)) == hipSuccess;
  mem_ok = mem_ok && h->comm_ids.reserve(n_total * sizeof(int32_t)) == hipSuccess;
  mem_ok = mem_ok && h->h_comm.reserve(rec_off + (size_t)world * n_total * sizeof(hgs_result)) == hipSuccess;
  if (!mem_ok) {
    hgs::comm_abort(h->comm);
    h->err = "hgs_loop_match_batch_sharded: no memory for the exchange buffers; the communicator has been aborted (the peers' collective fails instead of waiting)";
    return HGS_ERR_OUT_OF_MEMORY;
  }
  char err[256] = "";
  auto comm_failed = [&](const char* what) {
    h->err = std::string(what) + ": " + err;
    hgs::comm_abort(h->comm);
    return HGS_ERR_COMM;
  };
  std::vector<int32_t> counts(world, 0), statuses(world, 0);
  int32_t* h_hdr = static_cast<int32_t*>(h->h_comm.p);
  h_hdr[0] = (int32_t)n_send, h_hdr[1] = local, h_hdr[2] = 0, h_hdr[3] = 0;
  char* d_send = static_cast<char*>(h->comm_send.p);
  char* d_recv = static_cast<char*>(h->comm_recv.p);
  bool hip_ok = hipMemcpyAsync(d_send, h_hdr, hdr_bytes, hipMemcpyHostToDevice, h->stream) == hipSuccess;
  if (hgs::comm_all_gather(h->comm, d_send, d_recv, hdr_bytes, h->stream, err, sizeof(err)) != 0) return comm_failed("header all-gather");
  CommAbortGuard guard{h->comm};
  hip_ok = hip_ok && hipMemcpyAsync(h_hdr + 4, d_recv, (size_t)world * hdr_bytes, hipMemcpyDeviceToHost, h->stream) == hipSuccess;
  if (!h->comm_event) hip_ok = hip_ok && hipEventCreateWithFlags(&h->comm_event, hipEventDisableTiming) == hipSuccess;
  hip_ok = hip_ok && hipEventRecord(h->comm_event, h->stream) == hipSuccess;
  if (fault_after_header("guard", rank)) throw std::runtime_error("HGS_FAULT_AFTER_HEADER=guard");
  size_t n_valid = 0;
  if (n_send > 0 && hip_ok) {
    int rc;
    try {
      if (fault_after_header("batch", rank)) throw std::bad_alloc();
      rc = run_batch(h, src, guesses, &max_range);
    } catch (...) {
      rc = status_of_current_exception(h);
    }
    if (rc == HGS_OK) {
      n_valid = n_send;
    } else if (local == HGS_OK) {
      local = rc;
      try {
        local_err = h->err;
      } catch (...) {
      }
    }
  }
  if (hip_ok) {
    const int rc = comm_wait(h, [&] { return hipEventQuery(h->comm_event); }, "the gathered shard headers");
    if (rc != HGS_OK) {
      guard.armed = false;
      return rc;
    }
  }
  size_t per = 1;
  if (hip_ok)
    for (int r = 0; r < world; r++) {
      counts[r] = std::max(0, std::min<int32_t>(h_hdr[4 + 4 * r], (int32_t)n_total));
      statuses[r] = h_hdr[4 + 4 * r + 1];
      per = std::max(per, (size_t)counts[r]);
    }
  if (!hip_ok) {
    h->err = std::string("hgs_loop_match_batch_sharded: HIP error around the header exchange: ") + hipGetErrorString(hipGetLastError());
    return HGS_ERR_HIP;
  }
  hgs_result* d_records = reinterpret_cast<hgs_result*>(d_send + hdr_bytes);
  if (n_valid > 0) {
    std::memcpy(static_cast<char*>(h->h_comm.p) + ids_off, candidate_ids, n_valid * sizeof(int32_t));
    if (hipMemcpyAsync(h->comm_ids.p, static_cast<char*>(h->h_comm.p) + ids_off, n_valid * sizeof(int32_t), hipMemcpyHostToDevice, h->stream) != hipSuccess) n_valid = 0;
  }
  launch_results_to_records(h->stream, h->results.as<DevResult>(), h->comm_ids.as<int>(), (int)n_valid, (int)per, d_records);
  hgs_result* d_gathered = reinterpret_cast<hgs_result*>(d_recv + (size_t)world * hdr_bytes);
  if (hgs::comm_all_gather(h->comm, d_records, d_gathered, per * sizeof(hgs_result), h->stream, err, sizeof(err)) != 0) {
    guard.armed = false;
    return comm_failed("record all-gather");
  }
  guard.armed = false;
  hgs_result* gathered = reinterpret_cast<hgs_result*>(static_cast<char*>(h->h_comm.p) + rec_off);
  HGS_HIP(h, hipMemcpyAsync(gathered, d_gathered, (size_t)world * per * sizeof(hgs_result), hipMemcpyDeviceToHost, h->stream));
  HGS_TRY(comm_wait(h, [&] { return hipStreamQuery(h->stream); }, "the gathered records"));
  int32_t dup = -1;
  HGS_TRY(hgs_debug_merge_shard_records(gathered, counts.data(), world, per, n_total, all_out, &dup));
  if (best) HGS_TRY(hgs_select_best(all_out, n_total, best));
  if (local != HGS_OK) {
    h->err = local_err;
    return local;
  }
  if (dup >= 0) {
    h->err = "hgs_loop_match_batch_sharded: candidate id " + std::to_string(dup) + " was reported more than once (the first report was kept)";
    return HGS_ERR_INVALID_ARGUMENT;
  }
  h->err.clear();
  for (int r = 0; r < world; r++)
    if (statuses[r] != HGS_OK && r != rank) h->err += "rank " + std::to_string(r) + " reported status " + std::to_string(statuses[r]) + " (its candidates are not converged); ";
  return HGS_OK;
} catch (...) {
  return status_of_current_exception(h);
}

namespace {

int cloud_from_device(hgs_handle* h, const float4* src, size_t m, hgs_cloud** out) {
  hgs_cloud* c = nullptr;
  HGS_TRY(cloud_alloc(h, m, &c));
  const CloudDesc resident = resident_desc(c);
  launch_pf_to_cloud(h->stream, src, (int)m, const_cast<float4*>(c->desc.raw), c->intensity, c->desc.meta, &resident, c->dev_desc);
  launch_bbox_count(h->stream, c->dev_desc, 1, (int)m);
  hipError_t e = hipGetLastError();
  if (e != hipSuccess) {
    h->err = std::string("prefilter: building the resident cloud failed: ") + hipGetErrorString(e);
    cloud_free(c);
    return HGS_ERR_HIP;
  }
  *out = c;
  return HGS_OK;
}

}

extern "C" int hgs_prefilter_params_default(hgs_prefilter_params* p) try {
  if (!p) return HGS_ERR_INVALID_ARGUMENT;
  std::memset(p, 0, sizeof(*p));
  p->use_distance_filter = 1;
  p->distance_near_thresh = 1.0;
  p->distance_far_thresh = 100.0;
  p->downsample_method = HGS_DOWNSAMPLE_VOXELGRID;
  p->downsample_resolution = 0.1;
  p->outlier_removal_method = HGS_OUTLIER_STATISTICAL;
  p->statistical_mean_k = 20;
  p->statistical_stddev = 1.0;
  p->radius_radius = 0.8;
  p->radius_min_neighbors = 2;
  return HGS_OK;
} catch (...) {
  return status_of_current_exception(nullptr);
}

static bool prefilter_params_ok(const hgs_prefilter_params* p) {
  return !(p->downsample_method < HGS_DOWNSAMPLE_NONE || p->downsample_method > HGS_DOWNSAMPLE_APPROX_VOXELGRID || p->outlier_removal_method < HGS_OUTLIER_NONE ||
           p->outlier_removal_method > HGS_OUTLIER_RADIUS || (p->downsample_method != HGS_DOWNSAMPLE_NONE && !(p->downsample_resolution > 0)) ||
           (p->outlier_removal_method == HGS_OUTLIER_STATISTICAL && (p->statistical_mean_k < 1 || p->statistical_mean_k > 62)) ||
           (p->outlier_removal_method == HGS_OUTLIER_RADIUS && (!(p->radius_radius > 0) || p->radius_min_neighbors < 0)));
}
struct PfSweepArgs {
  float w[3] = {0.f, 0.f, 0.f};
  bool deskew = false, framed = false;
  double scan_period = 0.0;
  PfFrame frame{};
};
static int prefilter_sweep_args(hgs_handle* h, const void* pts, size_t n, size_t stride_bytes, const double* imu_angular_velocity, double scan_period,
                                const float* sensor_to_base, PfSweepArgs* a) {
  if ((n > 0 && !pts) || stride_bytes < 12 || (stride_bytes % 4) != 0 || n > (size_t)1 << 30) return HGS_ERR_INVALID_ARGUMENT;
  if (imu_angular_velocity) {
    if (!std::isfinite(scan_period)) return HGS_ERR_INVALID_ARGUMENT;
    for (int k = 0; k < 3; k++) a->w[k] = -(float)imu_angular_velocity[k];
    a->deskew = true, a->scan_period = scan_period;
  }
  if (sensor_to_base) {
    bool finite = true;
    for (int k = 0; k < 16; k++) finite = finite && std::isfinite(sensor_to_base[k]);
    if (!finite || sensor_to_base[3] != 0.f || sensor_to_base[7] != 0.f || sensor_to_base[11] != 0.f || sensor_to_base[15] != 1.f) {
      h->err = finite ? "prefilter: the bottom row of sensor_to_base is not 0 0 0 1" : "prefilter: sensor_to_base has a non-finite entry";
      return HGS_ERR_INVALID_ARGUMENT;
    }
    for (int r = 0; r < 3; r++)
      for (int c = 0; c < 4; c++) a->frame.rows[4 * r + c] = sensor_to_base[4 * c + r];
    a->framed = true;
  }
  return HGS_OK;
}

static int prefilter_impl(hgs_handle* h, const void* pts, size_t n, size_t stride_bytes, const hgs_prefilter_params* p, const double* imu_angular_velocity,
                          double scan_period, const float* sensor_to_base, hgs_cloud** out) {
  ApiLock lock(h);
  if (!h || !p || !out || !prefilter_params_ok(p)) return HGS_ERR_INVALID_ARGUMENT;
  PfSweepArgs args;
  HGS_TRY(prefilter_sweep_args(h, pts, n, stride_bytes, imu_angular_velocity, scan_period, sensor_to_base, &args));
  const float* deskew_w = args.deskew ? args.w : nullptr;
  scan_period = args.scan_period;
  const PfFrame* frame = args.framed ? &args.frame : nullptr;
  HGS_TRY(set_device(h));
  *out = nullptr;
  StageTimer tm(h, HGS_STAGE_PREFILTER);
  const size_t cap = std::max<size_t>(n, 1);
  HGS_HIP(h, h->pf_a.reserve(cap * sizeof(float4)));
  HGS_HIP(h, h->pf_b.reserve(cap * sizeof(float4)));
  HGS_HIP(h, h->pf_keep.reserve(cap * sizeof(uint32_t)));
  HGS_HIP(h, h->pf_slot.reserve(cap * sizeof(uint32_t)));
  HGS_HIP(h, h->pf_small.reserve(256));
  HGS_HIP(h, h->h_small.reserve(256));
  float4* cur = h->pf_a.as<float4>();
  float4* other = h->pf_b.as<float4>();
  bool grid_radius = false;
  int* d_count = h->pf_small.as<int>();
  unsigned* d_meta = h->pf_small.as<unsigned>() + 16;
  double* d_stats = reinterpret_cast<double*>(h->pf_small.as<char>() + 192);
  {
    const float4* staged = nullptr;
    if (n > 0) HGS_TRY(upload_points_packed(h, pts, n, stride_bytes, &staged));
    launch_pf_load(h->stream, staged, (int)n, cur, deskew_w, scan_period, frame, d_count, d_meta);
  }
  const bool voxelgrid = n > 0 && p->downsample_method == HGS_DOWNSAMPLE_VOXELGRID;
  const int inline_dist = (voxelgrid && p->use_distance_filter && h->prefilter_fast) ? 1 : 0;
  if (n > 0 && p->use_distance_filter && !inline_dist) {
    launch_pf_distance_flags(h->stream, cur, (int)n, 1, p->distance_near_thresh, p->distance_far_thresh, h->pf_keep.as<unsigned>());
    HGS_TRY(scan_u32(h, h->pf_keep.as<uint32_t>(), h->pf_slot.as<uint32_t>(), n));
    launch_pf_compact(h->stream, cur, (int)n, h->pf_keep.as<unsigned>(), h->pf_slot.as<unsigned>(), other, d_count);
    std::swap(cur, other);
  }
  if (n > 0 && p->downsample_method == HGS_DOWNSAMPLE_VOXELGRID) {
    const float inv_leaf = 1.0f / (float)p->downsample_resolution;
    launch_pf_bbox(h->stream, cur, d_count, (int)n, d_meta, inline_dist, p->distance_near_thresh, p->distance_far_thresh);
    launch_pf_grid(h->stream, d_meta, inv_leaf);
    HGS_TRY(reserve_sort_pairs(h, n));
    launch_pf_voxel_keys(h->stream, cur, d_count, d_meta, inv_leaf, (int)n, h->sort_keys[0].as<unsigned long long>(), h->sort_vals[0].as<unsigned>(), inline_dist,
                         p->distance_near_thresh, p->distance_far_thresh);
    HGS_TRY(sort_pairs(h, n, 0, 32));
    launch_pf_voxel_heads(h->stream, h->sort_keys[1].as<unsigned long long>(), (int)n, h->pf_keep.as<unsigned>(), kVoxelInvalidKey);
    HGS_TRY(scan_u32(h, h->pf_keep.as<uint32_t>(), h->pf_slot.as<uint32_t>(), n));
    grid_radius = h->prefilter_fast && p->outlier_removal_method == HGS_OUTLIER_RADIUS && p->radius_radius / p->downsample_resolution <= 4.0;
    unsigned* ukeys = nullptr;
    if (grid_radius) {
      HGS_HIP(h, h->pf_ukeys.reserve(n * sizeof(uint32_t)));
      ukeys = h->pf_ukeys.as<unsigned>();
// ... 1007 lines not shown
```

### hdl_graph_slam_amd/csrc/hgs_kernels.hip

```cpp
#include <hip/hip_runtime.h>
#include <type_traits>
#include "../../include/hgs_registration.h"
#include "hgs_device.h"
#include "hgs_wave_bvh.h"

namespace hgs {

#ifndef HGS_OPAQUE_POINTER
#define HGS_OPAQUE_POINTER(p) asm volatile("" : "+v"(p))
#define HGS_WAIT_VMEM() asm volatile("s_waitcnt vmcnt(0)" ::: "memory")
#define HGS_LANE_ID(dst) asm volatile("v_mbcnt_lo_u32_b32 %0, -1, 0\n\tv_mbcnt_hi_u32_b32 %0, -1, %0" : "=v"(dst))
#endif
#ifndef HGS_COMPILER_MEMORY_BARRIER
#define HGS_COMPILER_MEMORY_BARRIER() asm volatile("" ::: "memory")
#endif
#ifndef HGS_LOAD_GLOBAL_XYZ
__device__ __forceinline__ float4 hgs_load_global_xyz(const float4* p) {
  const __attribute__((address_space(1))) float* g = (const __attribute__((address_space(1))) float*)(p);
  return make_float4(g[0], g[1], g[2], 0.f);
}
#define HGS_LOAD_GLOBAL_XYZ(p) hgs_load_global_xyz(p)
#define HGS_OPAQUE_OFFSET(off) asm volatile("" : "+v"(off))
#define HGS_WAIT_VMEM_TRACKED() __builtin_amdgcn_s_waitcnt(0x0F70)
#endif
// ... 1123 lines not shown
  const float4 bp = jj >= 0 ? tgt.pts[jj] : make_float4(0.f, 0.f, 0.f, 0.f);
  if constexpr (RECIPROCAL) {
    const bool ractive = jj >= 0;
    if (__ballot(ractive) != 0ull) {
      const F3 r = icp_unmove_point(T, bp.x, bp.y, bp.z);
      BvhView sv;
      sv.nodes = d.nodes, sv.pts = d.pts, sv.lpts = d.lpts, sv.P = d.P, sv.n = n;
      float rd2;
      int rj, rorig;
      packet_nn1(sv, park[wave], r, ractive, c.search_bound2, ractive ? idx : -1, qpw, rd2, rj, rorig);
      if (ractive && !(rj >= 0 && rorig == __float_as_int(a.w) && (double)rd2 <= c.max_corr2)) jj = -1;
    }
  }
  if (active) __builtin_nontemporal_store(jj, d.corr + idx);
  double acc[kAccIcp];
  if (jj >= 0) {
    icp_pair_terms(q, bp.x, bp.y, bp.z, d2, acc);
  } else {
#pragma unroll
    for (int k = 0; k < kAccIcp; k++) acc[k] = 0.0;
  }
  int lane;
  HGS_LANE_ID(lane);
  int slot[kAccIcp];
#pragma unroll
  for (int k = 0; k < kAccIcp; k++) slot[k] = k;
  wave_sums_to<kAccIcp>(acc, slot, lds + wave * kAccIcp, lane);
  last_wave_stores<kAccIcp>(lds, &arrivals, partials + ((size_t)b * max_blocks + tile) * kAccIcp, lane);
}
void launch_icp_correspond(hipStream_t s, const CloudDesc* descs, TargetView tgt, const IcpState* states, IcpConsts c, double* partials, int max_blocks, int B) {
  if (c.reciprocal) hipLaunchKernelGGL(k_icp_correspond<true>, dim3(HGS_GRID_X(max_blocks), B), dim3(kBlock), 0, s, descs, tgt, states, c, partials, max_blocks);
  else hipLaunchKernelGGL(k_icp_correspond<false>, dim3(HGS_GRID_X(max_blocks), B), dim3(kBlock), 0, s, descs, tgt, states, c, partials, max_blocks);
}
void launch_icp_correspond(hipStream_t s, const CloudDesc* descs, const TargetView* tviews, const IcpState* states, IcpConsts c, double* partials, int max_blocks, int B) {
  if (c.reciprocal) hipLaunchKernelGGL((k_icp_correspond<true, const TargetView*>), dim3(HGS_GRID_X(max_blocks), B), dim3(kBlock), 0, s, descs, tviews, states, c, partials, max_blocks);
  else hipLaunchKernelGGL((k_icp_correspond<false, const TargetView*>), dim3(HGS_GRID_X(max_blocks), B), dim3(kBlock), 0, s, descs, tviews, states, c, partials, max_blocks);
}

__global__ __launch_bounds__(64) __attribute__((amdgpu_waves_per_eu(HGS_CONTROL_WAVES))) void k_icp_solve(const CloudDesc* descs, IcpState* states, IcpConsts c,
                                                                                        const double* __restrict__ partials, int max_blocks, Progress prog) {
  const int b = blockIdx.x;
  bool finished_now = false;
  if (HGS_CONTROL_PRIO) __builtin_amdgcn_s_setprio(HGS_CONTROL_PRIO);
  if (states[b].phase == ICP_RUN) {
    const int ntiles = (descs[b].meta->nvalid + kTileNN - 1) / kTileNN;
    const double* p = partials + (size_t)b * max_blocks * kAccIcp;
    double s[kAccIcp];
#pragma unroll
    for (int k = 0; k < kAccIcp; k++) s[k] = 0.0;
    for (int t = threadIdx.x; t < ntiles; t += 64)
#pragma unroll
      for (int k = 0; k < kAccIcp; k++) s[k] += p[(size_t)t * kAccIcp + k];
#pragma unroll
    for (int k = 0; k < kAccIcp; k++) s[k] = wave_sum(s[k]);
    if (threadIdx.x == 0) {
      IcpState st = states[b];
      icp_after_pass(st, s, c);
      states[b] = st;
      finished_now = st.phase == ICP_DONE;
    }
  }
  if (threadIdx.x == 0) progress_tick(prog, finished_now);
}
void launch_icp_solve(hipStream_t s, const CloudDesc* descs, IcpState* states, IcpConsts c, const double* partials, int max_blocks, int B, Progress prog) {
  hipLaunchKernelGGL(k_icp_solve, dim3(B), dim3(64), 0, s, descs, states, c, partials, max_blocks, prog);
}

__global__ void k_icp_results(const IcpState* states, DevResult* out, int B) {
  const int b = blockIdx.x * blockDim.x + threadIdx.x;
  if (b >= B) return;
  const IcpState st = states[b];
  DevResult r;
  pose_to_colmajor_f(st.x, r.T);
  r.converged = st.converged, r.iterations = st.iterations, r.lm_tries = st.passes, r.pad = 0;
  r.error = st.mse;
  r.fit_sum = 0, r.fit_count = 0, r.pad2 = 0;
  out[b] = r;
}
void launch_icp_results(hipStream_t s, const IcpState* states, DevResult* out, int B) {
  hipLaunchKernelGGL(k_icp_results, dim3((B + 63) / 64), dim3(64), 0, s, states, out, B);
}

template <typename TGT = TargetView>
__global__ __launch_bounds__(kBlock) __attribute__((amdgpu_waves_per_eu(HGS_FITNESS_WAVES))) void k_fitness(const CloudDesc* descs, TGT tgt_arg, const DevResult* poses, double max_range,
                                                    double* __restrict__ partials, int max_blocks, int use_seed, int qpw) {
  const int b = blockIdx.y;
  const TargetView& tgt = problem_target(tgt_arg, b);
  const CloudDesc d = descs[b];
  const int n = d.meta->nvalid;
  const int tile_pts = (kBlock / 64) * qpw * kNW;
  const int ntiles = (n + tile_pts - 1) / tile_pts;
  const int tile = xcd_tile(blockIdx.x, ntiles);
  if (tile >= ntiles) return;
  __shared__ double lds[4 * 2];
  __shared__ unsigned arrivals;
  __shared__ __attribute__((aligned(512))) float park[kBlock / 64][kParkFloats];
  if (threadIdx.x == 0) arrivals = 0u;
  __syncthreads();
  const int wave = __builtin_amdgcn_readfirstlane((int)(threadIdx.x >> 6));
  float Tf[12];
  const float* Tc = poses[b].T;
#pragma unroll
  for (int r = 0; r < 3; r++)
#pragma unroll
    for (int cc = 0; cc < 4; cc++) Tf[r * 4 + cc] = Tc[cc * 4 + r];
  const int idx = tile * tile_pts + wave * qpw + (int)(threadIdx.x & 63);
  const bool active = (int)(threadIdx.x & 63) < qpw && idx < n;
  const float4 a = active ? load_stream(d.pts + idx) : make_float4(0.f, 0.f, 0.f, 0.f);
  const F3 q = transform_point_f(Tf, a.x, a.y, a.z);
  int seed = (active && use_seed) ? __builtin_nontemporal_load(d.corr + idx) : -1;
  const BvhView tv = view_of(tgt);
  if (tgt.seed_bits && __ballot(active && !(seed >= 0 && seed < tv.n)) != 0ull) {
    if (active && !(seed >= 0 && seed < tv.n)) seed = seed_grid_lookup(tgt, q);
  }
  const bool seeded = seed >= 0 && seed < tv.n;
  float d2;
  int leaf;
  bool tie, found;
  if (__ballot(active && !seeded) != 0ull) wave_nn1_quad<true, false>(tv, park[wave], q, active, FLT_MAX, seed, qpw >> 1, d2, leaf, tie, found);
  else wave_nn1_quad<false, false>(tv, park[wave], q, active, FLT_MAX, seed, qpw >> 1, d2, leaf, tie, found);
  double acc[2] = {0.0, 0.0};
  if (active && found && (double)d2 <= max_range) acc[0] = (double)d2, acc[1] = 1.0;
  int lane;
  HGS_LANE_ID(lane);
  {
    const int slot[2] = {0, 1};
    wave_sums_to<2>(acc, slot, lds + wave * 2, lane);
  }
  last_wave_stores<2>(lds, &arrivals, partials + ((size_t)b * max_blocks + tile) * 2, lane);
}
void launch_fitness(hipStream_t s, const CloudDesc* descs, TargetView tgt, const DevResult* poses, double max_range, double* partials, int max_blocks,
                    int B, int use_seed, int qpw) {
  hipLaunchKernelGGL(k_fitness<TargetView>, dim3(HGS_GRID_X(max_blocks), B), dim3(kBlock), 0, s, descs, tgt, poses, max_range, partials, max_blocks, use_seed, qpw);
}
void launch_fitness(hipStream_t s, const CloudDesc* descs, const TargetView* tviews, const DevResult* poses, double max_range, double* partials, int max_blocks,
                    int B, int use_seed, int qpw) {
  hipLaunchKernelGGL(k_fitness<const TargetView*>, dim3(HGS_GRID_X(max_blocks), B), dim3(kBlock), 0, s, descs, tviews, poses, max_range, partials, max_blocks, use_seed, qpw);
}
__global__ __launch_bounds__(64) void k_fitness_final(const CloudDesc* descs, const double* __restrict__ partials, int max_blocks, DevResult* out, int tile_pts) {
  const int b = blockIdx.x;
  const int ntiles = (descs[b].meta->nvalid + tile_pts - 1) / tile_pts;
  double s = 0, c = 0;
  for (int t = threadIdx.x; t < ntiles; t += 64) {
    s += partials[((size_t)b * max_blocks + t) * 2];
    c += partials[((size_t)b * max_blocks + t) * 2 + 1];
  }
  s = wave_sum(s), c = wave_sum(c);
  if (threadIdx.x == 0) out[b].fit_sum = s, out[b].fit_count = (unsigned)(c + 0.5);
}
void launch_fitness_final(hipStream_t s, const CloudDesc* descs, const double* partials, int max_blocks, DevResult* out, int B, int tile_pts) {
  hipLaunchKernelGGL(k_fitness_final, dim3(B), dim3(64), 0, s, descs, partials, max_blocks, out, tile_pts);
}

__global__ void k_results_to_records(const DevResult* __restrict__ res, const int* __restrict__ candidate_ids, int n, int n_slots, hgs_result* __restrict__ out) {
  const int s = blockIdx.x * blockDim.x + threadIdx.x;
  if (s >= n_slots) return;
  hgs_result r;
  if (s < n) {
    const DevResult d = res[s];
#pragma unroll
    for (int k = 0; k < 16; k++) r.final_transformation[k] = d.T[k];
    r.converged = d.converged, r.iterations = d.iterations;
    r.error = d.error;
    r.num_inliers = d.fit_count;
    r.fitness_score = d.fit_count > 0 ? d.fit_sum / (double)d.fit_count : DBL_MAX;
    r.candidate_id = candidate_ids[s];
    r.lm_tries = d.lm_tries, r.reserved = 0;
  } else {
#pragma unroll
    for (int k = 0; k < 16; k++) r.final_transformation[k] = 0.f;
    r.converged = 0, r.iterations = 0, r.error = 0.0, r.fitness_score = DBL_MAX, r.num_inliers = 0, r.candidate_id = -1, r.lm_tries = 0, r.reserved = 0;
  }
  out[s] = r;
}
void launch_results_to_records(hipStream_t s, const DevResult* res, const int* candidate_ids, int n, int n_slots, hgs_result* out) {
  if (n_slots <= 0) return;
  hipLaunchKernelGGL(k_results_to_records, dim3((n_slots + 63) / 64), dim3(64), 0, s, res, candidate_ids, n, n_slots, out);
}

__global__ __launch_bounds__(kBlock) void k_nn_query(TargetView tgt, const float4* __restrict__ q, int nq, int* __restrict__ idx, float* __restrict__ d2out) {
  const int i = blockIdx.x * kBlock + threadIdx.x;
  if (i >= nq) return;
  const float4 p = q[i];
  float d2;
  int orig;
  const int j = bvh_nn1(view_of(tgt), F3{p.x, p.y, p.z}, FLT_MAX, &d2, &orig);
  idx[i] = j >= 0 ? orig : -1;
  d2out[i] = d2;
}
void launch_nn_query(hipStream_t s, TargetView tgt, const float4* q, int nq, int* idx, float* d2) {
  if (nq <= 0) return;
  hipLaunchKernelGGL(k_nn_query, dim3((nq + kBlock - 1) / kBlock), dim3(kBlock), 0, s, tgt, q, nq, idx, d2);
}

__global__ __launch_bounds__(kBlock) void k_transform(const float4* __restrict__ raw, int n, const float* __restrict__ T16, float4* __restrict__ out) {
  const int i = blockIdx.x * kBlock + threadIdx.x;
  if (i >= n) return;
  float Tf[12];
#pragma unroll
  for (int r = 0; r < 3; r++)
#pragma unroll
    for (int cc = 0; cc < 4; cc++) Tf[r * 4 + cc] = T16[cc * 4 + r];
  const float4 a = raw[i];
  const F3 q = transform_point_f(Tf, a.x, a.y, a.z);
  out[i] = make_float4(q.x, q.y, q.z, 1.0f);
}
void launch_transform(hipStream_t s, const float4* raw, int n, const float* T16_dev, float4* out) {
  if (n <= 0) return;
  hipLaunchKernelGGL(k_transform, dim3((n + kBlock - 1) / kBlock), dim3(kBlock), 0, s, raw, n, T16_dev, out);
}

__global__ void k_ndt_grid_params(CloudDesc d, float inv_leaf) {
  CloudMeta* m = d.meta;
  m->ndt_ncells = 0;
  m->ndt_error = 0;
  if (m->nvalid <= 0) {
    for (int k = 0; k < 3; k++) m->ndt_min_b[k] = 0, m->ndt_max_b[k] = -1, m->ndt_div_mul[k] = 0;
    return;
  }
  long long div[3];
  for (int k = 0; k < 3; k++) {
    m->ndt_min_b[k] = (int)floorf(ord2f(m->bbmin[k]) * inv_leaf);
    m->ndt_max_b[k] = (int)floorf(ord2f(m->bbmax[k]) * inv_leaf);
    div[k] = (long long)m->ndt_max_b[k] - m->ndt_min_b[k] + 1;
  }
  if (div[0] * div[1] * div[2] > 2147483647LL) m->ndt_error = 1;
  m->ndt_div_mul[0] = 1, m->ndt_div_mul[1] = (int)div[0], m->ndt_div_mul[2] = (int)(div[0] * div[1]);
}
void launch_ndt_grid_params(hipStream_t s, CloudDesc desc, float inv_leaf) { hipLaunchKernelGGL(k_ndt_grid_params, dim3(1), dim3(1), 0, s, desc, inv_leaf); }

__global__ __launch_bounds__(kBlock) void k_ndt_cell_keys(CloudDesc d, float inv_leaf, unsigned long long* __restrict__ keys, unsigned* __restrict__ vals) {
  const int i = blockIdx.x * kBlock + threadIdx.x;
  if (i >= d.n_input) return;
  const float4 p = d.raw[i];
  unsigned long long key = 0xffffffffull;
  const CloudMeta* m = d.meta;
  if (finite3(p) && !m->ndt_error) {
    const int cx = (int)floorf(p.x * inv_leaf) - m->ndt_min_b[0];
    const int cy = (int)floorf(p.y * inv_leaf) - m->ndt_min_b[1];
    const int cz = (int)floorf(p.z * inv_leaf) - m->ndt_min_b[2];
    key = (unsigned long long)(unsigned)(cx * m->ndt_div_mul[0] + cy * m->ndt_div_mul[1] + cz * m->ndt_div_mul[2]);
  }
  keys[i] = key;
  vals[i] = (unsigned)i;
}
void launch_ndt_cell_keys(hipStream_t s, CloudDesc desc, float inv_leaf, unsigned long long* keys, unsigned* vals) {
  if (desc.n_input <= 0) return;
  hipLaunchKernelGGL(k_ndt_cell_keys, dim3((desc.n_input + kBlock - 1) / kBlock), dim3(kBlock), 0, s, desc, inv_leaf, keys, vals);
}

__global__ __launch_bounds__(kBlock) void k_ndt_build_cells(CloudDesc d, const unsigned long long* __restrict__ keys, const unsigned* __restrict__ vals,
                                                            int min_points, int* hash_keys, int* hash_vals, int hash_mask, NdtCellRec* cells) {
  const int i = blockIdx.x * kBlock + threadIdx.x;
  if (i >= d.n_input) return;
  const unsigned long long key = keys[i];
  if (key == 0xffffffffull) return;
  if (i > 0 && keys[i - 1] == key) return;
  double sum[3] = {0, 0, 0};
  Sym3 sq = {0, 0, 0, 0, 0, 0};
  int n = 0;
  for (int j = i; j < d.n_input && keys[j] == key; j++) {
    const float4 p = d.raw[vals[j]];
    const double x = p.x, y = p.y, z = p.z;
    sum[0] += x, sum[1] += y, sum[2] += z;
    sq.xx += x * x, sq.xy += x * y, sq.xz += x * z, sq.yy += y * y, sq.yz += y * z, sq.zz += z * z;
    n++;
  }
  double mean[3];
  Sym3 icov;
  if (!ndt_finalize_cell(n, sum, sq, min_points, mean, &icov)) return;
  const int slot_c = atomicAdd(&d.meta->ndt_ncells, 1);
  NdtCellRec rec;
  rec.v0 = make_float4((float)icov.xx, (float)icov.xy, (float)icov.xz, (float)icov.yy);
  rec.v1 = make_float4((float)icov.yz, (float)icov.zz, (float)n, __int_as_float((int)key));
  rec.mean[0] = mean[0], rec.mean[1] = mean[1], rec.mean[2] = mean[2], rec.pad = 0.0;
  cells[slot_c] = rec;
  unsigned slot = (ndt_hash((int)key) >> 7) & (unsigned)hash_mask;
  for (;;) {
    const int prev = atomicCAS(&hash_keys[slot], -1, (int)key);
    if (prev == -1) {
      hash_vals[slot] = slot_c;
      break;
    }
    slot = (slot + 1) & (unsigned)hash_mask;
  }
}
void launch_ndt_build_cells(hipStream_t s, CloudDesc desc, const unsigned long long* sorted_keys, const unsigned* sorted_vals, int min_points,
                            int* hash_keys, int* hash_vals, int hash_mask, NdtCellRec* cells) {
  if (desc.n_input <= 0) return;
  hipLaunchKernelGGL(k_ndt_build_cells, dim3((desc.n_input + kBlock - 1) / kBlock), dim3(kBlock), 0, s, desc, sorted_keys, sorted_vals, min_points,
                     hash_keys, hash_vals, hash_mask, cells);
}

__global__ __launch_bounds__(64) void k_ndt_init(NdtState* states, NdtAngles* angles, const float* guesses, NdtConsts c, int B, Progress prog, NdtAccum* accum) {
  const int b = blockIdx.x;
  if (b == 0 && threadIdx.x == 0) prog.dev[0] = 0, prog.dev[1] = 0;
  if (accum) {
    static_assert(sizeof(NdtAccum) % sizeof(unsigned long long) == 0, "NdtAccum is zeroed word by word");
    unsigned long long* w = reinterpret_cast<unsigned long long*>(accum + b);
    for (int k = threadIdx.x; k < (int)(sizeof(NdtAccum) / sizeof(unsigned long long)); k += 64) w[k] = 0ull;
  }
  if (threadIdx.x == 0) {
    ndt_state_init(states[b], guesses + 16 * b);
    ndt_angle_tables(states[b].p, c.upstream_hd1_sign, angles[b]);
  }
}
void launch_ndt_init(hipStream_t s, NdtState* states, NdtAngles* angles, const float* guesses, NdtConsts c, int B, Progress prog, NdtAccum* accum_to_zero) {
  if (B <= 0) return;
  hipLaunchKernelGGL(k_ndt_init, dim3(B), dim3(64), 0, s, states, angles, guesses, c, B, prog, accum_to_zero);
}

__global__ __launch_bounds__(kBlock) void k_ndt_pack_hash(const int* __restrict__ keys, const int* __restrict__ vals, int2* __restrict__ kv, int cap) {
  const int i = blockIdx.x * kBlock + threadIdx.x;
  if (i >= cap) return;
  const int k = keys[i];
  kv[i] = make_int2(k, k == -1 ? -1 : vals[i]);
}
void launch_ndt_pack_hash(hipStream_t s, const int* keys, const int* vals, int2* kv, int cap) {
  hipLaunchKernelGGL(k_ndt_pack_hash, dim3((cap + kBlock - 1) / kBlock), dim3(kBlock), 0, s, keys, vals, kv, cap);
}

__device__ __forceinline__ void solve_svd6_wave(const double* A, const double* b, double* U, double* V, double* x) {
  const int lane = (int)(threadIdx.x & 63);
  if (lane < 36) U[lane] = A[lane], V[lane] = (lane % 7 == 0) ? 1.0 : 0.0;
  HGS_COMPILER_MEMORY_BARRIER();
  __builtin_amdgcn_wave_barrier();
  for (int sweep = 0; sweep < 60; sweep++) {
    bool rotated = false;
    for (int round = 0; round < 5; round++) {
      if (lane < 3) {
// ... 1584 lines not shown
```

### hdl_graph_slam_amd/registration.py

```python
from __future__ import annotations

import ctypes as C
import os

import numpy as np

from . import _lib as L


class HgsError(RuntimeError):
    pass


class DeviceCloud:

    def __init__(self, reg: "RegistrationHIP", cloud: np.ndarray):
        arr, n, stride = L.cloud_args(cloud)
        self._reg = reg
        self._h = C.c_void_p()
        reg._check(L.lib().hgs_cloud_create(reg._h, arr.ctypes.data_as(C.c_void_p), n, stride, C.byref(self._h)))
        self.size = n

    @classmethod
    def _adopt(cls, reg: "RegistrationHIP", handle) -> "DeviceCloud":
        self = cls.__new__(cls)
        self._reg, self._h = reg, handle
        self.size = int(L.lib().hgs_cloud_size(handle))
        return self

    def download(self) -> np.ndarray:
        from . import synth
        out = np.zeros(self.size, dtype=synth.POINT_XYZI_DTYPE)
        self._reg._check(L.lib().hgs_cloud_download(self._h, out.ctypes.data_as(C.c_void_p), out.dtype.itemsize))
        return out

    @property
    def device_bytes(self) -> int:
        return int(L.lib().hgs_cloud_device_bytes(self._h))

    def invalidate(self):
        L.lib().hgs_cloud_invalidate(self._h)

    def close(self):
        if self._h:
            self._reg._lib.hgs_cloud_destroy(self._h)
            self._h = C.c_void_p()

    def __del__(self):
        try:
            self.close()
        except Exception:
            pass


class _SearchMethodTarget:
    def __init__(self, reg):
        self._reg = reg

    def nearestKSearch(self, points: np.ndarray, k: int = 1):
        if k != 1:
            raise NotImplementedError("the callers only use k = 1 (scan_matching_odometry_nodelet.cpp:316)")
        arr, n, stride = L.cloud_args(points)
        idx = np.empty(n, np.int32)
        d2 = np.empty(n, np.float32)
        self._reg._check(L.lib().hgs_nn_target(self._reg._h, arr.ctypes.data_as(C.c_void_p), n, stride, idx.ctypes.data_as(C.c_void_p),
                                               d2.ctypes.data_as(C.c_void_p)))
        return idx, d2


class RegistrationHIP:
    def __init__(self, params: L.HgsParams):
        self.params = params
        self._h = C.c_void_p()
        self._lib = L.lib()
        rc = self._lib.hgs_create(C.byref(params), C.byref(self._h))
        if rc != L.HGS_OK:
            msg = L.lib().hgs_last_error(None)
            raise HgsError(f"hgs_create failed: {L.STATUS.get(rc, rc)}: {msg.decode() if msg else ''}")
        self._result = None
        self._source_n = 0
        self._source_stride = 0
        self._keep = {}
        for item in filter(None, os.environ.get("HGS_ENGINE_OPTIONS", "").split(",")):
            key, _, value = item.partition("=")
            self.set_option(key.strip(), int(value))

    def set_option(self, key: str, value: int):
        self._check(L.lib().hgs_debug_set_option(self._h, key.encode(), int(value)))

    def close(self):
        if self._h:
            self._lib.hgs_destroy(self._h)
            self._h = C.c_void_p()

    def __del__(self):
        try:
            self.close()
        except Exception:
            pass

    def _check(self, rc: int):
        if rc != L.HGS_OK:
            msg = L.lib().hgs_last_error(self._h)
            raise HgsError(f"{L.STATUS.get(rc, rc)}: {msg.decode() if msg else ''}")

    def setInputTarget(self, cloud):
        if isinstance(cloud, DeviceCloud):
            self._keep["t"] = cloud
            self._check(L.lib().hgs_set_target_cloud(self._h, cloud._h))
        else:
            arr, n, stride = L.cloud_args(cloud)
            self._check(L.lib().hgs_set_target(self._h, arr.ctypes.data_as(C.c_void_p), n, stride))

    def setInputSource(self, cloud):
        if isinstance(cloud, DeviceCloud):
            self._keep["s"] = cloud
            self._source_n = cloud.size
            self._check(L.lib().hgs_set_source_cloud(self._h, cloud._h))
        else:
            arr, n, stride = L.cloud_args(cloud)
            self._source_n = n
            self._check(L.lib().hgs_set_source(self._h, arr.ctypes.data_as(C.c_void_p), n, stride))

    def align(self, guess=None, return_cloud: bool = False):
        g = L.colmajor16(np.eye(4) if guess is None else guess)
        r = L.HgsResult()
        self._check(L.lib().hgs_align(self._h, L.fptr(g), C.byref(r)))
        self._result = r
        if return_cloud:
            return r, self.transformed_source(r.matrix())
        return r

    def transformed_source(self, T) -> np.ndarray:
        out = np.zeros((self._source_n, 4), np.float32)
        g = L.colmajor16(T)
        self._check(L.lib().hgs_transform_source(self._h, L.fptr(g), out.ctypes.data_as(C.c_void_p), 16))
        return out

    def hasConverged(self) -> bool:
        return bool(self._result.converged) if self._result is not None else False

    def getFinalTransformation(self) -> np.ndarray:
        return self._result.matrix() if self._result is not None else np.eye(4, dtype=np.float32)

    def getFitnessScore(self, max_range: float = L.DBL_MAX, T=None) -> float:
        g = L.colmajor16(self.getFinalTransformation() if T is None else T)
        score, ninl = C.c_double(), C.c_uint32()
        self._check(L.lib().hgs_fitness(self._h, L.fptr(g), float(max_range), C.byref(score), C.byref(ninl)))
        self.last_num_inliers = ninl.value
        return score.value

    def getSearchMethodTarget(self) -> _SearchMethodTarget:
        return _SearchMethodTarget(self)

    def upload(self, cloud) -> DeviceCloud:
        return DeviceCloud(self, cloud)

    def prefilter(self, cloud, params=None, imu_angular_velocity=None, scan_period: float = 0.1, base_link_transform=None) -> DeviceCloud:
        if params is None:
            params = L.HgsPrefilterParams()
            self._check(L.lib().hgs_prefilter_params_default(C.byref(params)))
        arr, n, stride = L.cloud_args(cloud)
        h = C.c_void_p()
        w = None if imu_angular_velocity is None else np.ascontiguousarray(imu_angular_velocity, np.float64).reshape(3)
        if base_link_transform is not None:
            m = L.colmajor16(base_link_transform)
            self._check(L.lib().hgs_prefilter_framed(self._h, arr.ctypes.data_as(C.c_void_p), n, stride, C.byref(params),
                                                     None if w is None else w.ctypes.data_as(C.c_void_p), float(scan_period), L.fptr(m), C.byref(h)))
        elif w is None:
            self._check(L.lib().hgs_prefilter(self._h, arr.ctypes.data_as(C.c_void_p), n, stride, C.byref(params), C.byref(h)))
        else:
            self._check(L.lib().hgs_prefilter_deskewed(self._h, arr.ctypes.data_as(C.c_void_p), n, stride, C.byref(params), w.ctypes.data_as(C.c_void_p),
                                                       float(scan_period), C.byref(h)))
        return DeviceCloud._adopt(self, h)

    def prefilter_batch(self, clouds, params=None, imu_angular_velocities=None, scan_periods=0.1, base_link_transforms=None) -> list:
        if params is None:
            params = L.HgsPrefilterParams()
            self._check(L.lib().hgs_prefilter_params_default(C.byref(params)))
        n = len(clouds)
        per = lambda v: [None] * n if v is None else list(v)
        ws, Ts = per(imu_angular_velocities), per(base_link_transforms)
        periods = [float(scan_periods)] * n if np.isscalar(scan_periods) else [float(x) for x in scan_periods]
        assert len(ws) == n and len(Ts) == n and len(periods) == n
        sweeps = (L.HgsPrefilterSweep * max(n, 1))()
        keep = []
        for i, cloud in enumerate(clouds):
            arr, m, stride = L.cloud_args(cloud)
            w = None if ws[i] is None else np.ascontiguousarray(ws[i], np.float64).reshape(3)
            T = None if Ts[i] is None else L.colmajor16(Ts[i])
            keep += [arr, w, T]
            sweeps[i].pts, sweeps[i].n, sweeps[i].stride_bytes, sweeps[i].scan_period = arr.ctypes.data, m, stride, periods[i]
            sweeps[i].imu_angular_velocity = None if w is None else w.ctypes.data
            sweeps[i].sensor_to_base = None if T is None else T.ctypes.data
        out = (C.c_void_p * max(n, 1))()
        self._check(L.lib().hgs_prefilter_batch(self._h, sweeps, n, C.byref(params), out))
        return [DeviceCloud._adopt(self, C.c_void_p(out[i])) for i in range(n)]

    def map_cloud(self, keyframes, poses, resolution: float) -> DeviceCloud:
        n = len(keyframes)
        arr = (C.c_void_p * max(n, 1))(*[k._h for k in keyframes])
        P = np.ascontiguousarray(np.stack([L.colmajor16(p) for p in poses]) if n else np.zeros((0, 16), np.float32))
        h = C.c_void_p()
        self._check(L.lib().hgs_map_cloud_generate(self._h, arr, P.ctypes.data_as(C.c_void_p), n, float(resolution), C.byref(h)))
        return DeviceCloud._adopt(self, h)

    def loop_match_batch(self, candidates, guesses, max_range: float = L.DBL_MAX):
        n = len(candidates)
        ptrs = (C.c_void_p * max(n, 1))(*[c._h for c in candidates])
        g = np.ascontiguousarray(np.stack([L.colmajor16(T) for T in guesses]) if n else np.zeros((0, 16), np.float32))
        out = np.zeros(n, dtype=L.RESULT_DTYPE)
        best = C.c_int32(-1)
        self._check(L.lib().hgs_loop_match_batch(self._h, ptrs, n, g.ctypes.data_as(C.c_void_p), float(max_range), out.ctypes.data_as(C.c_void_p),
                                                 C.byref(best)))
        return out, best.value

    def loop_match_groups(self, targets, groups, guesses, max_range: float = L.DBL_MAX, return_status: bool = False):
        ng = len(groups)
        offsets = np.zeros(ng + 1, np.uintp)
        offsets[1:] = np.cumsum([len(g) for g in groups])
        n = int(offsets[ng])
        tptr = (C.c_void_p * max(ng, 1))(*[(t._h if t is not None else None) for t in targets])
        cptr = (C.c_void_p * max(n, 1))(*[c._h for g in groups for c in g])
        flat = [L.colmajor16(T) for gg in guesses for T in gg]
        g = np.ascontiguousarray(np.stack(flat) if flat else np.zeros((0, 16), np.float32))
        out = np.zeros(n, dtype=L.RESULT_DTYPE)
        best = np.full(ng, -1, np.int32)
        rc = L.lib().hgs_loop_match_groups(self._h, tptr, ng, offsets.ctypes.data_as(C.c_void_p), cptr, g.ctypes.data_as(C.c_void_p), float(max_range),
                                           out.ctypes.data_as(C.c_void_p), best.ctypes.data_as(C.c_void_p))
        if return_status:
            return out, best, rc
        self._check(rc)
        return out, best

    def align_pairs(self, targets, sources, guesses, max_range=None, return_status: bool = False):
        n = len(sources)
        assert len(targets) == n and len(guesses) == n
        tptr = (C.c_void_p * max(n, 1))(*[(t._h if t is not None else None) for t in targets])
        sptr = (C.c_void_p * max(n, 1))(*[(s._h if s is not None else None) for s in sources])
        g = np.ascontiguousarray(np.stack([L.colmajor16(T) for T in guesses]) if n else np.zeros((0, 16), np.float32))
        out = np.zeros(n, dtype=L.RESULT_DTYPE)
# ... 156 lines not shown
```

### include/hgs_registration.h

```cpp
#ifndef HGS_REGISTRATION_H
#define HGS_REGISTRATION_H

#include <stddef.h>
#include <stdint.h>

#ifdef __cplusplus
extern "C" {
#endif

#define HGS_ABI_VERSION 5

enum hgs_status {
  HGS_OK = 0,
  HGS_ERR_INVALID_ARGUMENT = 1,
  HGS_ERR_NO_TARGET = 2,
  HGS_ERR_NO_SOURCE = 3,
  HGS_ERR_HIP = 4,
  HGS_ERR_NO_DEVICE = 5,
  HGS_ERR_UNSUPPORTED = 6,
  HGS_ERR_OUT_OF_MEMORY = 7,
  HGS_ERR_INTERNAL = 8,
  HGS_ERR_COMM = 9
};

// ... 50 lines not shown
  int32_t candidate_id;
  int32_t lm_tries;
  int32_t reserved;
} hgs_result;

typedef struct hgs_handle hgs_handle;
typedef struct hgs_cloud hgs_cloud;

int hgs_params_default(int32_t method, hgs_params* p);
int hgs_create(const hgs_params* p, hgs_handle** out);
int hgs_destroy(hgs_handle* h);
const char* hgs_last_error(const hgs_handle* h);
int hgs_abi_version(void);

int hgs_cloud_create(hgs_handle* h, const void* pts, size_t n, size_t stride_bytes, hgs_cloud** out);
int hgs_cloud_destroy(hgs_cloud* c);
size_t hgs_cloud_size(const hgs_cloud* c);
size_t hgs_cloud_device_bytes(const hgs_cloud* c);
int hgs_cloud_invalidate(hgs_cloud* c);

int hgs_set_target(hgs_handle* h, const void* pts, size_t n, size_t stride_bytes);
int hgs_set_target_cloud(hgs_handle* h, hgs_cloud* c);
int hgs_set_source(hgs_handle* h, const void* pts, size_t n, size_t stride_bytes);
int hgs_set_source_cloud(hgs_handle* h, hgs_cloud* c);
int hgs_align(hgs_handle* h, const float guess[16], hgs_result* out);
int hgs_transform_source(hgs_handle* h, const float T[16], void* out_pts, size_t stride_bytes);
int hgs_fitness(hgs_handle* h, const float T[16], double max_range, double* score, uint32_t* num_inliers);
int hgs_nn_target(hgs_handle* h, const float* q_xyz, size_t nq, size_t stride_bytes, int32_t* idx, float* d2);

int hgs_loop_match_batch(hgs_handle* h, hgs_cloud* const* candidates, size_t n_candidates, const float* guesses ,
                         double max_range, hgs_result* out, int32_t* best);
int hgs_loop_match_groups(hgs_handle* h, hgs_cloud* const* targets, size_t n_groups,
                          const size_t* group_offsets ,
                          hgs_cloud* const* candidates ,
                          const float* guesses ,
                          double max_range, hgs_result* out ,
                          int32_t* best );
int hgs_align_pairs(hgs_handle* h, hgs_cloud* const* targets , hgs_cloud* const* sources ,
                    const float* guesses , const double* max_range , size_t n,
                    hgs_result* out );
int hgs_select_best(const hgs_result* records, size_t n, int32_t* best);

#define HGS_COMM_UNIQUE_ID_BYTES 128
int hgs_comm_get_unique_id(void* id_out );
int hgs_comm_init(hgs_handle* h, int32_t rank, int32_t world, const void* unique_id );
int hgs_comm_finalize(hgs_handle* h);
int hgs_loop_match_batch_sharded(hgs_handle* h, hgs_cloud* const* candidates, size_t n_mine, const int32_t* candidate_ids,
                                 const float* guesses , size_t n_total, double max_range, hgs_result* all_out,
                                 int32_t* best);

int hgs_calc_fitness_score(hgs_handle* h, hgs_cloud* cloud1, hgs_cloud* cloud2, const float relpose[16], double max_range, double* score);
int hgs_calc_fitness_score_batch(hgs_handle* h, hgs_cloud* const* cloud1 , hgs_cloud* const* cloud2 ,
                                 const float* relposes , size_t n_pairs, double max_range,
                                 double* scores , uint32_t* num_inliers );

enum hgs_downsample_method { HGS_DOWNSAMPLE_NONE = 0, HGS_DOWNSAMPLE_VOXELGRID = 1, HGS_DOWNSAMPLE_APPROX_VOXELGRID = 2 };
enum hgs_outlier_removal { HGS_OUTLIER_NONE = 0, HGS_OUTLIER_STATISTICAL = 1, HGS_OUTLIER_RADIUS = 2 };
typedef struct hgs_prefilter_params {
  int32_t use_distance_filter;
  int32_t downsample_method;
  double distance_near_thresh;
  double distance_far_thresh;
  double downsample_resolution;
  int32_t outlier_removal_method;
  int32_t statistical_mean_k;
  double statistical_stddev;
  double radius_radius;
  int32_t radius_min_neighbors;
  int32_t reserved;
} hgs_prefilter_params;
int hgs_prefilter_params_default(hgs_prefilter_params* p);
int hgs_prefilter(hgs_handle* h, const void* pts, size_t n, size_t stride_bytes, const hgs_prefilter_params* p, hgs_cloud** out);
int hgs_prefilter_deskewed(hgs_handle* h, const void* pts, size_t n, size_t stride_bytes, const hgs_prefilter_params* p, const double* imu_angular_velocity,
                           double scan_period, hgs_cloud** out);
int hgs_prefilter_framed(hgs_handle* h, const void* pts, size_t n, size_t stride_bytes, const hgs_prefilter_params* p,
                         const double* imu_angular_velocity , double scan_period,
                         const float sensor_to_base[16] , hgs_cloud** out);
#define HGS_PREFILTER_BATCH_MAX_SWEEPS 4096
typedef struct hgs_prefilter_sweep {
  const void* pts;
  size_t n;
  size_t stride_bytes;
  const double* imu_angular_velocity;
  double scan_period;
  const float* sensor_to_base;
} hgs_prefilter_sweep;
int hgs_prefilter_batch(hgs_handle* h, const hgs_prefilter_sweep* sweeps, size_t n_sweeps, const hgs_prefilter_params* p, hgs_cloud** out );
int hgs_cloud_download(hgs_cloud* c, void* out_pts, size_t stride_bytes);

int hgs_map_cloud_generate(hgs_handle* h, hgs_cloud* const* keyframes, const float* poses, size_t n_keyframes, double resolution, hgs_cloud** out);

enum hgs_floor_reason {
  HGS_FLOOR_DETECTED = 0,
  HGS_FLOOR_TOO_FEW_POINTS = 1,
  HGS_FLOOR_TOO_FEW_INLIERS = 2,
  HGS_FLOOR_NOT_VERTICAL = 3
};
typedef struct hgs_floor_params {
  double tilt_deg;
  double sensor_height;
  double height_clip_range;
  int32_t floor_pts_thresh;
  int32_t use_normal_filtering;
  double floor_normal_thresh;
  double normal_filter_thresh;
  int32_t normal_k;
  int32_t ransac_max_iterations;
  double ransac_distance_threshold;
  double ransac_probability;
  uint32_t seed;
  int32_t reserved;
} hgs_floor_params;
typedef struct hgs_floor_result {
  float coeffs[4];
  int32_t detected;
  int32_t reason;
  uint32_t n_clipped;
  uint32_t n_filtered;
  uint32_t n_inliers;
  int32_t ransac_iterations;
} hgs_floor_result;
int hgs_floor_params_default(hgs_floor_params* p);
int hgs_detect_floor(hgs_handle* h, hgs_cloud* cloud, const hgs_floor_params* p, hgs_floor_result* out, hgs_cloud** filtered_out, hgs_cloud** inliers_out);

enum hgs_stage {
  HGS_STAGE_UPLOAD = 0,
  HGS_STAGE_INDEX = 1,
  HGS_STAGE_COVARIANCE = 2,
  HGS_STAGE_VOXELIZE = 3,
  HGS_STAGE_LINEARIZE = 4,
  HGS_STAGE_ERROR = 5,
  HGS_STAGE_SOLVE = 6,
  HGS_STAGE_FITNESS = 7,
  HGS_STAGE_PREFILTER = 8,
  HGS_STAGE_COUNT = 9
};
int hgs_profile_enable(hgs_handle* h, int enabled);
int hgs_profile_read(hgs_handle* h, double* ms, uint64_t* launches, int reset);
int hgs_synchronize(hgs_handle* h);

int hgs_debug_target_covariances(hgs_handle* h, float* out6);
int hgs_debug_gicp_linearize(hgs_handle* h, const double T12[12], double* H36, double* b6, double* err, int32_t* corr);
int hgs_debug_icp_correspond(hgs_handle* h, const double T12[12], double* sums17, int32_t* corr);
int hgs_debug_icp_step(hgs_handle* h, const double sums17[17], const double T12_in[12], double mse_prev, int32_t iterations_in,
                       double T12_out[12], int32_t flags3[3] , double* mse);
int hgs_debug_floor_filter(hgs_handle* h, hgs_cloud* cloud, const hgs_floor_params* p, uint8_t* keep_clip, uint8_t* keep_normal, double* normals3);
int hgs_debug_floor_ransac_counts(hgs_handle* h, hgs_cloud* cloud, const hgs_floor_params* p, uint32_t i0, uint32_t n, int32_t* counts, double* coeffs4);
int hgs_debug_ndt_cells(hgs_handle* h, int32_t cap, int32_t* ijk3, double* mean3, float* icov6, int32_t* npts, int32_t* n_cells);
int hgs_debug_vgicp_voxels(hgs_handle* h, int32_t cap, int32_t* ijk3, double* mean3, float* cov6, int32_t* npts, int32_t* n_cells);
int hgs_debug_cloud_seed_grid(hgs_handle* h, hgs_cloud* cloud, uint32_t* tab, size_t cap, int32_t* bits, size_t* entries);
int hgs_debug_ndt_derivatives(hgs_handle* h, const double p6[6], double* score, double* g6, double* H36);
int hgs_debug_merge_shard_records(const hgs_result* gathered, const int32_t* counts, int32_t world, size_t per, size_t n_total,
                                  hgs_result* all_out, int32_t* duplicate_id);
int hgs_debug_set_option(hgs_handle* h, const char* key, int32_t value);

#ifdef __cplusplus
}
#endif
#endif
```

Measured before the change: 5945 registrations/sec.

## Order batch problems by guess distance and run hardest half on priority streams

For GICP batches of at least eight problems, candidates are sorted on the host by the translation magnitude of their initial guess. The farther half goes to one or two high-priority HIP streams and the rest to normal lanes, and results are scattered back to the original order, including in the sharded record path. The aim is to start the longer-converging problems first so the batch tail is shorter and lanes finish closer together. The cost is extra host sorting and copying, extra streams, and a lane planner capped at four lanes that may use fewer lanes than before.

```diff
diff --git a/hdl_graph_slam_amd/_lib.py b/hdl_graph_slam_amd/_lib.py
--- a/hdl_graph_slam_amd/_lib.py
+++ b/hdl_graph_slam_amd/_lib.py
@@ -108,6 +108,7 @@
     "hgs_floor_params_default", "hgs_detect_floor", "hgs_debug_floor_filter", "hgs_debug_floor_ransac_counts",
     "hgs_profile_enable", "hgs_profile_read", "hgs_synchronize",
     "hgs_debug_target_covariances", "hgs_debug_gicp_linearize", "hgs_debug_icp_correspond", "hgs_debug_icp_step", "hgs_debug_ndt_cells", "hgs_debug_vgicp_voxels", "hgs_debug_cloud_seed_grid", "hgs_debug_ndt_derivatives", "hgs_debug_merge_shard_records", "hgs_debug_set_option",
+    "hgs_debug_lane_plan", "hgs_debug_plan_lanes", "hgs_debug_batch_order",
 ]
 
 _lib = None
@@ -168,6 +169,9 @@
     L.hgs_synchronize.argtypes = [vp]
     L.hgs_debug_target_covariances.argtypes = [vp, vp]
     L.hgs_debug_set_option.argtypes = [vp, C.c_char_p, C.c_int32]
+    L.hgs_debug_lane_plan.argtypes = [vp, C.POINTER(C.c_int32), C.POINTER(C.c_int32), C.POINTER(C.c_int32)]
+    L.hgs_debug_plan_lanes.argtypes = [vp, C.c_int32, C.c_int32, C.c_int32, C.c_int32, C.POINTER(C.c_int32), C.POINTER(C.c_int32)]
+    L.hgs_debug_batch_order.argtypes = [vp, C.POINTER(C.c_int32), C.c_int32, C.POINTER(C.c_int32)]
     L.hgs_debug_gicp_linearize.argtypes = [vp, vp, vp, vp, vp, vp]
     L.hgs_debug_icp_correspond.argtypes = [vp, vp, vp, vp]
     L.hgs_debug_icp_step.argtypes = [vp, vp, vp, C.c_double, C.c_int32, vp, vp, vp]
diff --git a/hdl_graph_slam_amd/csrc/hgs_device.h b/hdl_graph_slam_amd/csrc/hgs_device.h
--- a/hdl_graph_slam_amd/csrc/hgs_device.h
+++ b/hdl_graph_slam_amd/csrc/hgs_device.h
@@ -136,7 +136,7 @@
 }
 struct hgs_result;
 namespace hgs {
-void launch_results_to_records(hipStream_t s, const DevResult* res, const int* candidate_ids, int n, int n_slots, ::hgs_result* out);
+void launch_results_to_records(hipStream_t s, const DevResult* res, const int* candidate_ids, const int* pos, int n, int n_slots, ::hgs_result* out);
 void launch_nn_query(hipStream_t s, TargetView tgt, const float4* q, int nq, int* idx, float* d2);
 void launch_seed_grid_build(hipStream_t s, const float4* pts, const CloudMeta* meta, int n_max, unsigned* tab, int bits);
 inline size_t seed_grid_entries(int bits) { return ((size_t)1 << bits) + ((size_t)1 << (bits - 2)) + ((size_t)1 << (bits - 4)); }
diff --git a/hdl_graph_slam_amd/csrc/hgs_engine.hip b/hdl_graph_slam_amd/csrc/hgs_engine.hip
--- a/hdl_graph_slam_amd/csrc/hgs_engine.hip
+++ b/hdl_graph_slam_amd/csrc/hgs_engine.hip
@@ -87,6 +87,10 @@
   hipStream_t stream = nullptr;
   hipStream_t lane_stream[7] = {};
   hipEvent_t lane_event[8] = {};
+  int lane_order = 1;
+  hipStream_t prio_stream[2] = {};
+  std::vector<int> batch_order;
+  int last_lanes = 0, last_ahead_lanes = 0;
   int lane_start = 1;
   int nn_qpw = 0;
   int nn_qpw16_below = 96, nn_qpw32_below = 0;
@@ -159,6 +163,8 @@
   void synchronize_streams() {
     if (stream) (void)hipStreamSynchronize(stream);
     for (hipStream_t ls : lane_stream)
+      if (ls) (void)hipStreamSynchronize(ls);
+    for (hipStream_t ls : prio_stream)
       if (ls) (void)hipStreamSynchronize(ls);
   }
   ~hgs_handle();
@@ -704,51 +710,85 @@
   bool finished = false;
 };
 
-int open_lanes(hgs_handle* h, int B, size_t partial_bytes_per_problem, size_t partial_err_bytes_per_problem, std::vector<BatchLane>& lanes, int tiles_per_problem) {
+struct LanePlan {
+  int lanes, ahead;
+};
+LanePlan plan_lanes(hgs_handle* h, int B, int tiles_per_problem, bool ordered, int assume_streams = -1) {
   const bool small_problems = tiles_per_problem > 0 && tiles_per_problem <= 96;
   const int by_size = h->prm.method == HGS_NDT_OMP ? (B > 32 && !small_problems ? 3 : 4) : (small_problems && (long)B * tiles_per_problem <= 3072 ? 1 : 4);
   const int wanted = h->batch_lanes > 0 ? h->batch_lanes : by_size;
   int n = h->profiling ? 1 : std::max(1, std::min(std::min(wanted, kMaxLanes), B));
-  if (h->batch_lanes <= 0) {
-    int owned = 0;
-    while (owned < kMaxLanes - 1 && h->lane_stream[owned]) owned++;
-    const int room = std::max(0, hw_queue_budget() - streams_in_use(h->device).load(std::memory_order_relaxed));
-    n = std::min(n, 1 + owned + room);
-  }
+  int owned = 0, owned_prio = 0;
+  while (owned < kMaxLanes - 1 && h->lane_stream[owned]) owned++;
+  while (owned_prio < 2 && h->prio_stream[owned_prio]) owned_prio++;
+  const int room = std::max(0, hw_queue_budget() - (assume_streams >= 0 ? assume_streams : streams_in_use(h->device).load(std::memory_order_relaxed)));
+  const int plain = h->batch_lanes <= 0 ? std::min(n, 1 + owned + room) : n;
+  if (!ordered || h->profiling || plain < 2) return LanePlan{plain, 0};
+  n = std::min(n, 4);
+  auto ahead_of = [](int lanes) { return lanes >= 4 ? 2 : 1; };
+  if (h->batch_lanes <= 0)
+    while (n > 1 && std::max(0, ahead_of(n) - owned_prio) + std::max(0, n - ahead_of(n) - 1 - owned) > room) n--;
+  if (n < 2 || n < std::min(plain, 4)) return LanePlan{plain, 0};
+  return LanePlan{n, ahead_of(n)};
+}
+
+hipError_t create_priority_stream(hipStream_t* out) {
+#ifdef HGS_SIMT_EMULATION
+  return hipStreamCreateWithFlags(out, hipStreamNonBlocking);
+#else
+  int least = 0, greatest = 0;
+  const hipError_t e = hipDeviceGetStreamPriorityRange(&least, &greatest);
+  if (e != hipSuccess) return e;
+  return hipStreamCreateWithPriority(out, hipStreamNonBlocking, greatest);
+#endif
+}
+
+int open_lanes(hgs_handle* h, int B, size_t partial_bytes_per_problem, size_t partial_err_bytes_per_problem, std::vector<BatchLane>& lanes, int tiles_per_problem,
+               int ahead_problems = 0) {
+  const LanePlan plan = plan_lanes(h, B, tiles_per_problem, ahead_problems > 0);
+  const int n = plan.lanes;
+  h->last_lanes = n, h->last_ahead_lanes = plan.ahead;
   lanes.assign(n, BatchLane{});
-  for (int i = 0, b0 = 0; i < n; i++) {
+  for (int i = 0, b0 = 0, extra = 0; i < n; i++) {
     BatchLane& L = lanes[i];
-    L.b0 = b0, L.B = (B - b0) / (n - i);
+    const bool ahead = i < plan.ahead;
+    const int group_end = plan.ahead == 0 ? B : (ahead ? ahead_problems : B), group_lanes_left = plan.ahead == 0 ? n - i : (ahead ? plan.ahead - i : n - i);
+    L.b0 = b0, L.B = (group_end - b0) / group_lanes_left;
     b0 += L.B;
     HGS_TRY(make_progress(h, i, L.B, &L.prog));
-    if (i == 0) {
+    if (i == plan.ahead) {
       L.stream = h->stream;
       L.partials = h->partials.as<double>(), L.partials_err = h->partials_err.as<double>();
       continue;
     }
-    if (!h->lane_stream[i - 1]) {
-      HGS_HIP(h, hipStreamCreateWithFlags(&h->lane_stream[i - 1], hipStreamNonBlocking));
+    hipStream_t& ls = ahead ? h->prio_stream[i] : h->lane_stream[i - plan.ahead - 1];
+    if (!ls) {
+      HGS_HIP(h, ahead ? create_priority_stream(&ls) : hipStreamCreateWithFlags(&ls, hipStreamNonBlocking));
       streams_in_use(h->device).fetch_add(1, std::memory_order_relaxed);
     }
-    L.stream = h->lane_stream[i - 1];
-    HGS_HIP(h, h->lane_partials[i - 1].reserve((size_t)L.B * partial_bytes_per_problem));
-    HGS_HIP(h, h->lane_partials_err[i - 1].reserve((size_t)L.B * partial_err_bytes_per_problem));
-    L.partials = h->lane_partials[i - 1].as<double>(), L.partials_err = h->lane_partials_err[i - 1].as<double>();
+    L.stream = ls;
+    HGS_HIP(h, h->lane_partials[extra].reserve((size_t)L.B * partial_bytes_per_problem));
+    HGS_HIP(h, h->lane_partials_err[extra].reserve((size_t)L.B * partial_err_bytes_per_problem));
+    L.partials = h->lane_partials[extra].as<double>(), L.partials_err = h->lane_partials_err[extra].as<double>();
+    extra++;
   }
   if (n > 1) {
     if (h->lane_start != 0) HGS_HIP(h, hipStreamSynchronize(h->stream));
     if (!h->lane_event[0]) HGS_HIP(h, hipEventCreateWithFlags(&h->lane_event[0], hipEventDisableTiming));
     HGS_HIP(h, hipEventRecord(h->lane_event[0], h->stream));
-    for (int i = 1; i < n; i++) HGS_HIP(h, hipStreamWaitEvent(lanes[i].stream, h->lane_event[0], 0));
+    for (BatchLane& L : lanes)
+      if (L.stream != h->stream) HGS_HIP(h, hipStreamWaitEvent(L.stream, h->lane_event[0], 0));
   }
   return HGS_OK;
 }
 
 int close_lanes(hgs_handle* h, std::vector<BatchLane>& lanes) {
-  for (size_t i = 1; i < lanes.size(); i++) {
-    if (!h->lane_event[i]) HGS_HIP(h, hipEventCreateWithFlags(&h->lane_event[i], hipEventDisableTiming));
-    HGS_HIP(h, hipEventRecord(h->lane_event[i], lanes[i].stream));
-    HGS_HIP(h, hipStreamWaitEvent(h->stream, h->lane_event[i], 0));
+  for (size_t i = 0; i < lanes.size(); i++) {
+    if (lanes[i].stream == h->stream) continue;
+    const size_t ev = i == 0 ? lanes.size() : i;
+    if (!h->lane_event[ev]) HGS_HIP(h, hipEventCreateWithFlags(&h->lane_event[ev], hipEventDisableTiming));
+    HGS_HIP(h, hipEventRecord(h->lane_event[ev], lanes[i].stream));
+    HGS_HIP(h, hipStreamWaitEvent(h->stream, h->lane_event[ev], 0));
   }
   return HGS_OK;
 }
@@ -841,7 +881,7 @@
   if (fit_max_range) lane_fitness(h, L, s, *fit_max_range, corr_seeds_fitness(h->prm.method));
 }
 
-int run_gicp_rounds(hgs_handle* h, const BatchShape& s, const float* guesses_host, bool guess_in_args, const double* fit_max_range) {
+int run_gicp_rounds(hgs_handle* h, const BatchShape& s, const float* guesses_host, bool guess_in_args, const double* fit_max_range, int ahead_problems = 0) {
   const int B = s.B, max_blocks = s.max_blocks;
   hgs_cloud* tgt = h->target;
   const bool voxel = h->prm.method == HGS_FAST_VGICP;
@@ -861,7 +901,7 @@
   const NdtTargetView vtv = voxel && !s.d_vviews ? vgicp_target_view(tgt) : NdtTargetView{};
   const long max_rounds = (long)std::max(1, c.max_iterations) * std::max(1, c.lm_max_iterations) + 2 + (round2 ? 1 : 0);
   std::vector<BatchLane> lanes;
-  HGS_TRY(open_lanes(h, B, (size_t)max_blocks * kAccNdt * sizeof(double), (size_t)max_blocks * 2 * sizeof(double), lanes, s.err_blocks));
+  HGS_TRY(open_lanes(h, B, (size_t)max_blocks * kAccNdt * sizeof(double), (size_t)max_blocks * 2 * sizeof(double), lanes, s.err_blocks, ahead_problems));
   auto finish_lane = [&](BatchLane& L) {
     if (early && *L.prog.host_done) {
       h->early_valid = true;
@@ -1028,9 +1068,23 @@
   return close_lanes(h, lanes);
 }
 
+constexpr int kLaneOrderMinProblems = 8;
+void lane_order_of(const float* guesses, int B, std::vector<int>& order) {
+  std::vector<float> hint(B);
+  for (int b = 0; b < B; b++) {
+    const float* t = guesses + (size_t)b * 16 + 12;
+    const float d2 = t[0] * t[0] + t[1] * t[1] + t[2] * t[2];
+    hint[b] = std::isfinite(d2) ? d2 : FLT_MAX;
+  }
+  order.resize(B);
+  for (int b = 0; b < B; b++) order[b] = b;
+  std::stable_sort(order.begin(), order.end(), [&](int a, int b) { return hint[a] > hint[b]; });
+}
+
 int run_batch(hgs_handle* h, const std::vector<hgs_cloud*>& sources, const float* guesses_host, const double* fit_max_range = nullptr) {
   const int B = (int)sources.size();
   h->early_valid = false;
+  h->batch_order.clear();
   hgs_cloud* tgt = h->target;
   const int method = h->prm.method;
   const bool gicp = method == HGS_FAST_GICP || method == HGS_FAST_VGICP;
@@ -1051,15 +1105,32 @@
     HGS_TRY(ensure_ndt_target(h, tgt));
   }
   if (fit_max_range && method != HGS_FAST_GICP) HGS_TRY(ensure_seed_grid(h, tgt));
+  std::vector<hgs_cloud*> ordered_sources;
+  std::vector<float> ordered_guesses;
+  int ahead_problems = 0;
+  if (gicp && h->lane_order && B >= kLaneOrderMinProblems) {
+    int max_n = 0;
+    for (hgs_cloud* c : sources) max_n = std::max(max_n, (int)c->n_input);
+    if (plan_lanes(h, B, std::max(1, (max_n + kBlock - 1) / kBlock) , true).ahead > 0) {
+      lane_order_of(guesses_host, B, h->batch_order);
+      ordered_sources.resize(B), ordered_guesses.resize((size_t)B * 16);
+      for (int i = 0; i < B; i++) {
+        ordered_sources[i] = sources[h->batch_order[i]];
+        std::memcpy(&ordered_guesses[(size_t)i * 16], guesses_host + (size_t)h->batch_order[i] * 16, 16 * sizeof(float));
+      }
+      guesses_host = ordered_guesses.data();
+      ahead_problems = (B + 1) / 2;
+    }
+  }
   BatchShape s;
-  HGS_TRY(batch_shape(h, sources, true, &s));
+  HGS_TRY(batch_shape(h, ahead_problems ? ordered_sources : sources, true, &s));
   const bool guess_in_args = B == 1 && method == HGS_FAST_GICP;
   HGS_HIP(h, h->guesses.reserve((size_t)B * 16 * sizeof(float)));
   if (!guess_in_args) HGS_HIP(h, h->up.upload(h->guesses.p, guesses_host, (size_t)B * 16 * sizeof(float), h->stream));
   HGS_HIP(h, h->results.reserve((size_t)B * sizeof(DevResult)));
   HGS_HIP(h, h->partials.reserve((size_t)B * s.max_blocks * kAccNdt * sizeof(double)));
   HGS_HIP(h, h->partials_err.reserve((size_t)B * s.max_blocks * 2 * sizeof(double)));
-  if (gicp) HGS_TRY(run_gicp_rounds(h, s, guesses_host, guess_in_args, fit_max_range));
+  if (gicp) HGS_TRY(run_gicp_rounds(h, s, guesses_host, guess_in_args, fit_max_range, ahead_problems));
   else if (method == HGS_ICP) HGS_TRY(run_icp_rounds(h, s, fit_max_range));
   else HGS_TRY(run_ndt_rounds(h, sources, s, fit_max_range));
   HGS_HIP(h, hipGetLastError());
@@ -1070,6 +1141,7 @@
   const int B = (int)sources.size();
   const int method = h->prm.method;
   h->early_valid = false;
+  h->batch_order.clear();
   std::vector<hgs_cloud*> all(sources);
   all.insert(all.end(), targets.begin(), targets.end());
   if (method == HGS_FAST_GICP) HGS_TRY(ensure_cov(h, all, h->prm.correspondence_randomness));
@@ -1106,6 +1178,7 @@
   const int B = (int)sources.size();
   const bool voxel = method == HGS_FAST_VGICP;
   h->early_valid = false;
+  h->batch_order.clear();
   std::vector<hgs_cloud*> all(sources);
   all.insert(all.end(), targets.begin(), targets.end());
   std::vector<hgs_cloud*> distinct;
@@ -1180,6 +1253,8 @@
   HGS_HIP(h, hipMemcpyAsync(h->h_results.p, h->results.p, (size_t)B * sizeof(DevResult), hipMemcpyDeviceToHost, h->stream));
   HGS_HIP(h, hipStreamSynchronize(h->stream));
   out.assign(h->h_results.as<DevResult>(), h->h_results.as<DevResult>() + B);
+  if ((int)h->batch_order.size() == B)
+    for (int i = 0; i < B; i++) out[h->batch_order[i]] = h->h_results.as<DevResult>()[i];
   return HGS_OK;
 }
 
@@ -1207,6 +1282,7 @@
     std::memset(poses.data(), 0, B * sizeof(DevResult));
     for (size_t b = 0; b < B; b++) std::memcpy(poses[b].T, relposes + 16 * (p0 + b), sizeof(float) * 16);
     HGS_HIP(h, h->results.reserve(B * sizeof(DevResult)));
+    h->batch_order.clear();
     HGS_HIP(h, h->up.upload(h->results.p, poses.data(), B * sizeof(DevResult), h->stream));
     HGS_HIP(h, h->partials_err.reserve(B * s.max_blocks * 2 * sizeof(double)));
     BatchLane whole;
@@ -1238,6 +1314,7 @@
 }
 
 int upload_pose_as_result(hgs_handle* h, const float T[16]) {
+  h->batch_order.clear();
   HGS_HIP(h, h->results.reserve(sizeof(DevResult)));
   HGS_HIP(h, h->h_results.reserve(sizeof(DevResult)));
   DevResult* r = h->h_results.as<DevResult>();
@@ -1301,6 +1378,8 @@
     for (const ProfEvent& ev : *list) (void)hipEventDestroy(ev.a), (void)hipEventDestroy(ev.b);
   for (hipStream_t ls : lane_stream)
     if (ls) (void)hipStreamDestroy(ls), streams_in_use(device).fetch_sub(1, std::memory_order_relaxed);
+  for (hipStream_t ls : prio_stream)
+    if (ls) (void)hipStreamDestroy(ls), streams_in_use(device).fetch_sub(1, std::memory_order_relaxed);
   if (stream) (void)hipStreamDestroy(stream), streams_in_use(device).fetch_sub(1, std::memory_order_relaxed);
 }
 
@@ -1314,6 +1393,7 @@
   const std::string k(key);
   if (k == "batch_lanes") h->batch_lanes = value <= 0 ? 0 : std::min(kMaxLanes, value);
   else if (k == "lane_start") h->lane_start = value != 0 ? 1 : 0;
+  else if (k == "lane_order") h->lane_order = value != 0 ? 1 : 0;
   else if (k == "ndt_sort") h->ndt_sort = std::max(-1, std::min(1, value));
   else if (k == "cov_split") h->cov_split = value != 0 ? 1 : 0;
   else if (k == "fused_rounds") h->fused_rounds = value != 0 ? 1 : 0;
@@ -1346,6 +1426,38 @@
   return status_of_current_exception(h);
 }
 
+int hgs_debug_lane_plan(hgs_handle* h, int32_t* lanes, int32_t* ahead_lanes, int32_t* process_streams) try {
+  ApiLock lock(h);
+  if (!h) return HGS_ERR_INVALID_ARGUMENT;
+  if (lanes) *lanes = h->last_lanes;
+  if (ahead_lanes) *ahead_lanes = h->last_ahead_lanes;
+  if (process_streams) *process_streams = streams_in_use(h->device).load(std::memory_order_relaxed);
+  return HGS_OK;
+} catch (...) {
+  return status_of_current_exception(h);
+}
+
+int hgs_debug_plan_lanes(hgs_handle* h, int32_t n_problems, int32_t tiles_per_problem, int32_t ordered, int32_t assume_streams, int32_t* lanes, int32_t* ahead_lanes) try {
+  ApiLock lock(h);
+  if (!h || n_problems < 1) return HGS_ERR_INVALID_ARGUMENT;
+  const LanePlan plan = plan_lanes(h, n_problems, tiles_per_problem, ordered != 0 && h->lane_order && n_problems >= kLaneOrderMinProblems, assume_streams);
+  if (lanes) *lanes = plan.lanes;
+  if (ahead_lanes) *ahead_lanes = plan.ahead;
+  return HGS_OK;
+} catch (...) {
+  return status_of_current_exception(h);
+}
+
+int hgs_debug_batch_order(hgs_handle* h, int32_t* order, int32_t cap, int32_t* n) try {
+  ApiLock lock(h);
+  if (!h || !n || cap < 0 || (cap > 0 && !order)) return HGS_ERR_INVALID_ARGUMENT;
+  *n = (int32_t)h->batch_order.size();
+  for (int32_t i = 0; i < std::min(cap, *n); i++) order[i] = h->batch_order[i];
+  return HGS_OK;
+} catch (...) {
+  return status_of_current_exception(h);
+}
+
 int hgs_params_default(int32_t method, hgs_params* p) try {
   if (!p || method < HGS_FAST_GICP || method > HGS_ICP) return HGS_ERR_INVALID_ARGUMENT;
   std::memset(p, 0, sizeof(*p));
@@ -1937,12 +2049,12 @@
   }
   const size_t n_send = local == HGS_OK ? n_mine : 0;
   const size_t hdr_bytes = 16;
-  const size_t ids_off = align_up((size_t)world * hdr_bytes + hdr_bytes, 16), rec_off = align_up(ids_off + n_total * sizeof(int32_t), 16);
+  const size_t ids_off = align_up((size_t)world * hdr_bytes + hdr_bytes, 16), rec_off = align_up(ids_off + 2 * n_total * sizeof(int32_t), 16);
   bool mem_ok = set_device(h) == HGS_OK;
   mem_ok = mem_ok && h->results.reserve(std::max<size_t>(n_total, 1) * sizeof(DevResult)) == hipSuccess;
   mem_ok = mem_ok && h->comm_send.reserve(n_total * sizeof(hgs_result) + hdr_bytes) == hipSuccess;
   mem_ok = mem_ok && h->comm_recv.reserve((size_t)world * (n_total * sizeof(hgs_result) + hdr_bytes)) == hipSuccess;
-  mem_ok = mem_ok && h->comm_ids.reserve(n_total * sizeof(int32_t)) == hipSuccess;
+  mem_ok = mem_ok && h->comm_ids.reserve(2 * n_total * sizeof(int32_t)) == hipSuccess;
   mem_ok = mem_ok && h->h_comm.reserve(rec_off + (size_t)world * n_total * sizeof(hgs_result)) == hipSuccess;
   if (!mem_ok) {
     hgs::comm_abort(h->comm);
@@ -2005,11 +2117,16 @@
     return HGS_ERR_HIP;
   }
   hgs_result* d_records = reinterpret_cast<hgs_result*>(d_send + hdr_bytes);
+  const bool ordered = n_valid > 0 && h->batch_order.size() == n_valid;
   if (n_valid > 0) {
-    std::memcpy(static_cast<char*>(h->h_comm.p) + ids_off, candidate_ids, n_valid * sizeof(int32_t));
-    if (hipMemcpyAsync(h->comm_ids.p, static_cast<char*>(h->h_comm.p) + ids_off, n_valid * sizeof(int32_t), hipMemcpyHostToDevice, h->stream) != hipSuccess) n_valid = 0;
-  }
-  launch_results_to_records(h->stream, h->results.as<DevResult>(), h->comm_ids.as<int>(), (int)n_valid, (int)per, d_records);
+    int32_t* h_ids = reinterpret_cast<int32_t*>(static_cast<char*>(h->h_comm.p) + ids_off);
+    std::memcpy(h_ids, candidate_ids, n_valid * sizeof(int32_t));
+    if (ordered)
+      for (size_t i = 0; i < n_valid; i++) h_ids[n_valid + (size_t)h->batch_order[i]] = (int32_t)i;
+    if (hipMemcpyAsync(h->comm_ids.p, h_ids, (ordered ? 2 : 1) * n_valid * sizeof(int32_t), hipMemcpyHostToDevice, h->stream) != hipSuccess) n_valid = 0;
+  }
+  launch_results_to_records(h->stream, h->results.as<DevResult>(), h->comm_ids.as<int>(), ordered && n_valid > 0 ? h->comm_ids.as<int>() + n_valid : nullptr, (int)n_valid,
+                            (int)per, d_records);
   hgs_result* d_gathered = reinterpret_cast<hgs_result*>(d_recv + (size_t)world * hdr_bytes);
   if (hgs::comm_all_gather(h->comm, d_records, d_gathered, per * sizeof(hgs_result), h->stream, err, sizeof(err)) != 0) {
     guard.armed = false;
diff --git a/hdl_graph_slam_amd/csrc/hgs_kernels.hip b/hdl_graph_slam_amd/csrc/hgs_kernels.hip
--- a/hdl_graph_slam_amd/csrc/hgs_kernels.hip
+++ b/hdl_graph_slam_amd/csrc/hgs_kernels.hip
@@ -1299,12 +1299,13 @@
   hipLaunchKernelGGL(k_fitness_final, dim3(B), dim3(64), 0, s, descs, partials, max_blocks, out, tile_pts);
 }
 
-__global__ void k_results_to_records(const DevResult* __restrict__ res, const int* __restrict__ candidate_ids, int n, int n_slots, hgs_result* __restrict__ out) {
+__global__ void k_results_to_records(const DevResult* __restrict__ res, const int* __restrict__ candidate_ids, const int* __restrict__ pos, int n, int n_slots,
+                                     hgs_result* __restrict__ out) {
   const int s = blockIdx.x * blockDim.x + threadIdx.x;
   if (s >= n_slots) return;
   hgs_result r;
   if (s < n) {
-    const DevResult d = res[s];
+    const DevResult d = res[pos ? pos[s] : s];
 #pragma unroll
     for (int k = 0; k < 16; k++) r.final_transformation[k] = d.T[k];
     r.converged = d.converged, r.iterations = d.iterations;
@@ -1320,9 +1321,9 @@
   }
   out[s] = r;
 }
-void launch_results_to_records(hipStream_t s, const DevResult* res, const int* candidate_ids, int n, int n_slots, hgs_result* out) {
+void launch_results_to_records(hipStream_t s, const DevResult* res, const int* candidate_ids, const int* pos, int n, int n_slots, hgs_result* out) {
   if (n_slots <= 0) return;
-  hipLaunchKernelGGL(k_results_to_records, dim3((n_slots + 63) / 64), dim3(64), 0, s, res, candidate_ids, n, n_slots, out);
+  hipLaunchKernelGGL(k_results_to_records, dim3((n_slots + 63) / 64), dim3(64), 0, s, res, candidate_ids, pos, n, n_slots, out);
 }
 
 __global__ __launch_bounds__(kBlock) void k_nn_query(TargetView tgt, const float4* __restrict__ q, int nq, int* __restrict__ idx, float* __restrict__ d2out) {
diff --git a/hdl_graph_slam_amd/registration.py b/hdl_graph_slam_amd/registration.py
--- a/hdl_graph_slam_amd/registration.py
+++ b/hdl_graph_slam_amd/registration.py
@@ -87,6 +87,23 @@
 
     def set_option(self, key: str, value: int):
         self._check(L.lib().hgs_debug_set_option(self._h, key.encode(), int(value)))
+
+    def lane_plan(self):
+        lanes, ahead, streams = C.c_int32(), C.c_int32(), C.c_int32()
+        self._check(L.lib().hgs_debug_lane_plan(self._h, C.byref(lanes), C.byref(ahead), C.byref(streams)))
+        return lanes.value, ahead.value, streams.value
+
+    def plan_lanes(self, n_problems: int, tiles_per_problem: int, ordered: bool = True, assume_streams: int = -1):
+        lanes, ahead = C.c_int32(), C.c_int32()
+        self._check(L.lib().hgs_debug_plan_lanes(self._h, int(n_problems), int(tiles_per_problem), int(bool(ordered)), int(assume_streams), C.byref(lanes), C.byref(ahead)))
+        return lanes.value, ahead.value
+
+    def batch_order(self):
+        n = C.c_int32()
+        self._check(L.lib().hgs_debug_batch_order(self._h, None, 0, C.byref(n)))
+        buf = (C.c_int32 * max(1, n.value))()
+        self._check(L.lib().hgs_debug_batch_order(self._h, buf, n.value, C.byref(n)))
+        return list(buf[:n.value])
 
     def close(self):
         if self._h:
diff --git a/include/hgs_registration.h b/include/hgs_registration.h
--- a/include/hgs_registration.h
+++ b/include/hgs_registration.h
@@ -226,6 +226,9 @@
 int hgs_debug_ndt_derivatives(hgs_handle* h, const double p6[6], double* score, double* g6, double* H36);
 int hgs_debug_merge_shard_records(const hgs_result* gathered, const int32_t* counts, int32_t world, size_t per, size_t n_total,
                                   hgs_result* all_out, int32_t* duplicate_id);
+int hgs_debug_lane_plan(hgs_handle* h, int32_t* lanes, int32_t* ahead_lanes, int32_t* process_streams);
+int hgs_debug_plan_lanes(hgs_handle* h, int32_t n_problems, int32_t tiles_per_problem, int32_t ordered, int32_t assume_streams, int32_t* lanes, int32_t* ahead_lanes);
+int hgs_debug_batch_order(hgs_handle* h, int32_t* order, int32_t cap, int32_t* n);
 int hgs_debug_set_option(hgs_handle* h, const char* key, int32_t value);
 
 #ifdef __cplusplus
```

After: 6094 registrations/sec (median of 6 runs). 1.03x the previous value.
